# r9y9/gantts

Measured on NVIDIA H100. Metric: gan_step_frames_per_sec, higher is better.
Workload: dtype f32 (GEMMs: bf16x3 split on wgmma, fp32 accumulate)

## Files before the change

### gantts_b200/csrc/common.cuh

```cuda
#pragma once
#include <cuda_runtime.h>
#include <stdint.h>
#include <stdio.h>
#include <stdlib.h>
#include <string.h>

#include "../../include/gantts_b200.h"

namespace gantts {

void set_error(const char* fmt, ...);
int cuda_fail(cudaError_t e, const char* what);

#define GANTTS_CHECK_ARG(cond, ...)            \
  do {                                         \
    if (!(cond)) {                             \
      ::gantts::set_error(__VA_ARGS__);        \
      return GANTTS_E_BADARG;                  \
    }                                          \
  } while (0)

#define GANTTS_CUDA(call)                                        \
  do {                                                           \
    cudaError_t _e = (call);                                     \
    if (_e != cudaSuccess) return ::gantts::cuda_fail(_e, #call); \
  } while (0)

#define GANTTS_LAUNCH_CHECK(name)                                     \
  do {                                                                \
    cudaError_t _e = cudaGetLastError();                              \
    if (_e != cudaSuccess) return ::gantts::cuda_fail(_e, "launch " name); \
    ::gantts::count_launch();                                         \
  } while (0)

void count_launch();
enum ProfKind { PROF_GEMM_KK = 0, PROF_GEMM_MN = 1, PROF_MLPG_FWD = 2, PROF_MLPG_BWD = 3, PROF_LSTM_FWD = 4,
                PROF_LSTM_BWD = 5, PROF_WORLD_RESPONSE = 6, PROF_WORLD_OLA = 7, PROF_KINDS = 8 };
void prof_begin(int kind, double work, cudaStream_t st);
void prof_end(cudaStream_t st);

static inline cudaStream_t as_stream(void* s) { return reinterpret_cast<cudaStream_t>(s); }

int side_stream(cudaStream_t* out);
int stream_wait(cudaStream_t waiter, cudaStream_t on);

__device__ __forceinline__ void pdl_entry() {
  asm volatile("griddepcontrol.launch_dependents;" ::: "memory");
  asm volatile("griddepcontrol.wait;" ::: "memory");
}
inline int pdl_enabled() {
  static int v = -1;
  if (v < 0) {
    const char* e = getenv("GANTTS_B200_PDL");
    v = e ? atoi(e) : 1;
  }
  return v;
}
template <typename... KA, typename... A>
static inline void pdl_launch(void (*kern)(KA...), dim3 grid, dim3 block, size_t smem, cudaStream_t st, A&&... args) {
  cudaLaunchConfig_t cfg = {};
  cfg.gridDim = grid;
  cfg.blockDim = block;
  cfg.dynamicSmemBytes = smem;
  cfg.stream = st;
  cudaLaunchAttribute at[1];
  at[0].id = cudaLaunchAttributeProgrammaticStreamSerialization;
  at[0].val.programmaticStreamSerializationAllowed = 1;
  cfg.attrs = at;
  cfg.numAttrs = pdl_enabled() ? 1 : 0;
  cudaLaunchKernelEx(&cfg, kern, static_cast<KA>(args)...);
}
#define GANTTS_PDL_LAUNCH(kern, grid, block, smem, st, ...) \
  ::gantts::pdl_launch(kern, dim3(grid), dim3(block), (size_t)(smem), st, __VA_ARGS__)

__device__ __forceinline__ float warp_sum(float v) {
#pragma unroll
  for (int o = 16; o > 0; o >>= 1) v += __shfl_xor_sync(0xffffffffu, v, o);
  return v;
}

template <int NV>
__device__ __forceinline__ void block_sum(float (&v)[NV], float* smem) {
  const int lane = threadIdx.x & 31, warp = threadIdx.x >> 5, nwarp = (blockDim.x + 31) >> 5;
#pragma unroll
  for (int i = 0; i < NV; ++i) v[i] = warp_sum(v[i]);
  if (lane == 0) {
#pragma unroll
    for (int i = 0; i < NV; ++i) smem[i * 32 + warp] = v[i];
  }
  __syncthreads();
  if (warp == 0) {
#pragma unroll
    for (int i = 0; i < NV; ++i) {
      float x = lane < nwarp ? smem[i * 32 + lane] : 0.f;
      v[i] = warp_sum(x);
    }
  }
}

__device__ __forceinline__ void fft_radix2_stages(double2* z, const double2* w, int N) {
  for (int h = 1; h < N; h <<= 1) {
    const int step = N / h;
    for (int i = threadIdx.x; i < N / 2; i += blockDim.x) {
      const int pos = i & (h - 1), i0 = ((i - pos) << 1) + pos, i1 = i0 + h;
      const double2 tw = w[pos * step], a = z[i0], v = z[i1];
      const double tr = tw.x * v.x - tw.y * v.y, ti = tw.x * v.y + tw.y * v.x;
      z[i0] = make_double2(a.x + tr, a.y + ti);
      z[i1] = make_double2(a.x - tr, a.y - ti);
    }
    __syncthreads();
  }
}

__device__ __forceinline__ double2 rfft_split(const double2* z, const double2* w, int k, int N) {
  if (k == 0 || k == N)
    return make_double2(k == 0 ? z[0].x + z[0].y : z[0].x - z[0].y, 0.0);
  const double2 a = z[k], c = z[N - k];
  const double er = 0.5 * (a.x + c.x), ei = 0.5 * (a.y - c.y);
  const double orr = 0.5 * (a.y + c.y), oi = -0.5 * (a.x - c.x);
  const double2 tw = w[k];
  return make_double2(er + (tw.x * orr - tw.y * oi), ei + (tw.x * oi + tw.y * orr));
}

struct DropBits {
  uint32_t a, b;
};
__device__ __forceinline__ DropBits dropout_quad_bits(uint64_t seed, uint32_t row, uint32_t quarter_n, uint32_t quad) {
  uint32_t x = (row * quarter_n + quad) * 0x9E3779B1u + static_cast<uint32_t>(seed);
  x ^= x >> 16; x *= 0x7feb352dU; x ^= x >> 15; x *= 0x846ca68bU; x ^= x >> 16;
  uint32_t y = x * 0x9E3779B1u;
  y ^= y >> 15;
  const uint32_t s = static_cast<uint32_t>(seed >> 32);
  DropBits r;
  r.a = x ^ s;
  r.b = y ^ s;
  return r;
}
__device__ __forceinline__ uint32_t drop_limit(uint32_t thresh) { return ((thresh - 1u) << 16) | 0xffffu; }
__device__ __forceinline__ bool dropout_keep(uint64_t seed, uint32_t row, uint32_t n_cols, uint32_t col,
                                             uint32_t thresh) {
  const DropBits q = dropout_quad_bits(seed, row, (n_cols + 3) >> 2, col >> 2);
  const uint32_t w = (col & 2) ? q.b : q.a;
  const uint32_t f = (col & 1) ? (w >> 16) : (w & 0xffffu);
  return f >= thresh;
}

}
```

### gantts_b200/csrc/core.cu

```cuda
#include <stdarg.h>

#include <mutex>
#include <vector>

#include "common.cuh"

namespace gantts {
static thread_local char g_err[512] = "";

void set_error(const char* fmt, ...) {
  va_list ap;
  va_start(ap, fmt);
  vsnprintf(g_err, sizeof(g_err), fmt, ap);
  va_end(ap);
}

int cuda_fail(cudaError_t e, const char* what) {
  set_error("CUDA error %d (%s) in %s", static_cast<int>(e), cudaGetErrorString(e), what);
  return GANTTS_E_CUDA;
}

static long long g_launches = 0;
void count_launch() { ++g_launches; }

struct ProfRec {
  cudaEvent_t e0, e1;
  int kind;
  double work;
};
static bool g_prof_on = false;
static std::vector<ProfRec> g_recs;
static std::vector<cudaEvent_t> g_pool;
static ProfRec g_open;
static bool g_open_valid = false;

static cudaEvent_t get_event() {
  cudaEvent_t e;
  if (!g_pool.empty()) {
    e = g_pool.back();
    g_pool.pop_back();
    return e;
  }
  cudaEventCreate(&e);
  return e;
}

void prof_begin(int kind, double work, cudaStream_t st) {
  if (!g_prof_on) return;
  g_open.e0 = get_event();
  g_open.e1 = get_event();
  g_open.kind = kind;
  g_open.work = work;
  cudaEventRecord(g_open.e0, st);
  g_open_valid = true;
}

void prof_end(cudaStream_t st) {
  if (!g_prof_on || !g_open_valid) return;
  cudaEventRecord(g_open.e1, st);
  g_recs.push_back(g_open);
  g_open_valid = false;
}

struct SideStream {
  cudaStream_t st = nullptr;
  cudaEvent_t ev = nullptr;
};
static std::mutex g_side_mu;
static SideStream g_side[64];

static int side_locked(SideStream** out) {
  int dev = 0;
  GANTTS_CUDA(cudaGetDevice(&dev));
  GANTTS_CHECK_ARG(dev >= 0 && dev < 64, "side stream: device ordinal %d out of range", dev);
  SideStream& s = g_side[dev];
  if (!s.ev) GANTTS_CUDA(cudaEventCreateWithFlags(&s.ev, cudaEventDisableTiming));
  if (!s.st) {
    int least = 0, greatest = 0;
    GANTTS_CUDA(cudaDeviceGetStreamPriorityRange(&least, &greatest));
    GANTTS_CUDA(cudaStreamCreateWithPriority(&s.st, cudaStreamNonBlocking, greatest));
  }
  *out = &s;
  return GANTTS_OK;
}

int side_stream(cudaStream_t* out) {
  std::lock_guard<std::mutex> lk(g_side_mu);
  SideStream* s;
  int rc = side_locked(&s);
  if (rc) return rc;
  *out = s->st;
  return GANTTS_OK;
}

int stream_wait(cudaStream_t waiter, cudaStream_t on) {
  std::lock_guard<std::mutex> lk(g_side_mu);
  SideStream* s;
  int rc = side_locked(&s);
  if (rc) return rc;
  GANTTS_CUDA(cudaEventRecord(s->ev, on));
  GANTTS_CUDA(cudaStreamWaitEvent(waiter, s->ev, 0));
  return GANTTS_OK;
}
}

extern "C" long long gantts_launch_count(void) { return gantts::g_launches; }

extern "C" int gantts_profile_enable(int on) {
  gantts::g_prof_on = on != 0;
  return GANTTS_OK;
}

extern "C" int gantts_profile_collect(double* ms, double* work, long long* launches) {
  using namespace gantts;
  for (auto& r : g_recs) {
    float t = 0.f;
    cudaError_t e = cudaEventSynchronize(r.e1);
    if (e == cudaSuccess) e = cudaEventElapsedTime(&t, r.e0, r.e1);
    if (e != cudaSuccess) return cuda_fail(e, "profile_collect");
    if (r.kind >= 0 && r.kind < PROF_KINDS) {
      if (ms) ms[r.kind] += t;
      if (work) work[r.kind] += r.work;
      if (launches) launches[r.kind] += 1;
    }
    g_pool.push_back(r.e0);
    g_pool.push_back(r.e1);
  }
  g_recs.clear();
  return GANTTS_OK;
}

extern "C" int gantts_version(void) { return 104; }

extern "C" const char* gantts_last_error_string(void) { return gantts::g_err; }

extern "C" int gantts_device_supported(void) {
  int dev = 0;
  if (cudaGetDevice(&dev) != cudaSuccess) return 0;
  cudaDeviceProp prop;
  if (cudaGetDeviceProperties(&prop, dev) != cudaSuccess) return 0;
  return (prop.major == 9 && prop.minor == 0) ? 1 : 0;
}
```

### gantts_b200/csrc/gan_step.cu

```cuda
#include <nvtx3/nvToolsExt.h>

#include "common.cuh"

namespace gantts {

struct NvtxRange {
  explicit NvtxRange(const char* name) { nvtxRangePushA(name); }
  ~NvtxRange() { nvtxRangePop(); }
};

enum ScalarSlot {
  S_REAL = 0,
  S_FAKE = 3,
  S_ADV = 6,
  S_MGE = 9,
  S_MSE = 11,
  S_DSUMSQ = 13,
  S_GSUMSQ = 14,
  S_INV_T = 15,
  S_ADV_SCALE = 16,
  S_MGE_SCALE = 17,
  S_MSE_SCALE = 18,
  S_COUNT = 32
};
// ... 610 lines not shown
    w->c[l] = a.f32((size_t)M * nc);
    if (l < nl - 1) w->h[l] = a.f32((size_t)M * nc);
    w->w[l] = a.take(2 * plane_bytes(ni, ku) + 2 * plane_bytes(ku, ni));
    w->partial[l] = reinterpret_cast<float*>(a.take(mn_partial_bytes_upto(M, ni, ku)));
  }
  w->du = a.take(nl > 0 ? 2 * plane_bytes(M, maxku) : 0);
  w->dx = a.f32((size_t)M * nc);
  w->dxp = a.f32((size_t)M * nc);
  w->bpart = a.f32((size_t)c->B * 2 * nc);
}

static Planes sru_in_planes(const gantts_gan_step_t* c, const StepLayout& L, int l, int64_t M) {
  char* cur = L.sru.in[l];
  return carve_planes(cur, M, sru_nin(c->sru, l));
}
static void sru_w_planes(const gantts_gan_step_t* c, const StepLayout& L, int l, Planes* w, Planes* wt) {
  const int ni = sru_nin(c->sru, l), ku = sru_ncols(c->sru) * sru_k(c->sru, l);
  char* cur = L.sru.w[l];
  *w = carve_planes(cur, ni, ku);
  *wt = carve_planes(cur, ku, ni);
}

static int sru_stack_fwd(const gantts_gan_step_t* c, const gantts_mlp_t& g, const ParamList& pg, const StepLayout& L,
                         const float* x, int B, int T, uint64_t seed, bool train, cudaStream_t st) {
  const int64_t M = (int64_t)B * T;
  const gantts_sru_stack_t& s = c->sru;
  const int nl = s.num_layers, nc = sru_ncols(s);
  const float p_h = train ? s.dropout : 0.f, p_x = train ? s.rnn_dropout : 0.f;
  int rc;
  {
    WeightSplitList wl;
    wl.n = nl;
    wl.off[0] = 0;
    for (int l = 0; l < nl; ++l) {
      Planes w, wt;
      sru_w_planes(c, L, l, &w, &wt);
      wl.W[l] = pg.sru[l][WEIGHT].p;
      wl.N[l] = (int)w.rows;
      wl.K[l] = (int)w.cols;
      wl.hi[l] = w.hi;
      wl.lo[l] = w.lo;
      wl.pitch[l] = w.pitch;
      wl.thi[l] = wt.hi;
      wl.tlo[l] = wt.lo;
      wl.tpitch[l] = wt.pitch;
      wl.off[l + 1] = wl.off[l] + (int64_t)((w.rows + 31) / 32) * ((w.cols + 31) / 32);
    }
    int nb = (int)(wl.off[nl] < num_sms() * 8 ? wl.off[nl] : num_sms() * 8);
    GANTTS_PDL_LAUNCH((split_weights_kernel), nb < 1 ? 1 : nb, 256, 0, st, wl);
    GANTTS_LAUNCH_CHECK("split_weights_kernel(sru)");
  }
  const Planes in0 = sru_in_planes(c, L, 0, M);
  if (p_x > 0.f) {
    GANTTS_PDL_LAUNCH((sru_mask_split_kernel), blocks_1d(M * s.in_dim, 1024), 256, 0, st, x, (int64_t)s.in_dim, M, s.in_dim,
                      T, sru_mask(gantts_sru_mask_seed(seed, 0, 0), p_x), in0.hi, in0.lo, in0.pitch);
    GANTTS_LAUNCH_CHECK("sru_mask_split_kernel");
  } else if ((rc = launch_split(x, s.in_dim, M, s.in_dim, in0, 0, st))) {
    return rc;
  }
  Planes top;
  if ((rc = mlp_tape_input_planes(&g, M, L.g_tape, L.g_tape_bytes, &top))) return rc;
  for (int l = 0; l < nl; ++l) {
    const int k = sru_k(s, l);
    const bool last = l == nl - 1;
    Planes w, wt;
    sru_w_planes(c, L, l, &w, &wt);
    EpiArgs e;
    e.epi = EPI_F32;
    e.C = L.sru.u[l];
    e.ldc = (int64_t)nc * k;
    if ((rc = launch_gemm_kk(sru_in_planes(c, L, l, M), wt, e, st))) return rc;
    const Planes out = last ? top : sru_in_planes(c, L, l + 1, M);
    SruStepFwd p{};
    p.u = L.sru.u[l];
    p.xh = k == 3 ? (l == 0 ? x : L.sru.h[l - 1]) : nullptr;
    p.xh_rs = l == 0 ? s.in_dim : nc;
    p.bias = pg.sru[l][BIAS].p;
    p.c = L.sru.c[l];
    p.h = L.sru.h[l];
    p.hi = out.hi;
    p.lo = out.lo;
    p.pitch = out.pitch;
    p.mh = sru_mask(gantts_sru_mask_seed(seed, l, 1), last ? 0.f : p_h);
    p.mx = sru_mask(gantts_sru_mask_seed(seed, l + 1, 0), last ? 0.f : p_x);
    p.B = B;
    p.T = T;
    p.d = s.hidden;
    p.bidir = s.bidirectional;
    p.act = s.act;
    if ((rc = launch_sru_step_fwd(p, k, st))) return rc;
  }
  return GANTTS_OK;
}

static int sru_stack_bwd(const gantts_gan_step_t* c, const StepLayout& L, const ParamList& pg, const float* x, int B, int T,
                         uint64_t seed, cudaStream_t st) {
  const int64_t M = (int64_t)B * T;
  const gantts_sru_stack_t& s = c->sru;
  const int nl = s.num_layers, nc = sru_ncols(s);
  int rc;
  ReduceList rl;
  for (int l = nl - 1; l >= 0; --l) {
    const int k = sru_k(s, l);
    const bool top = l == nl - 1;
    char* cur = L.sru.du;
    const Planes du = carve_planes(cur, M, (int64_t)nc * k);
    SruStepBwd p{};
    p.u = L.sru.u[l];
    p.xh = k == 3 ? (l == 0 ? x : L.sru.h[l - 1]) : nullptr;
    p.xh_rs = l == 0 ? s.in_dim : nc;
    p.bias = pg.sru[l][BIAS].p;
    p.c = L.sru.c[l];
    p.dx = L.sru.dx;
    p.dxp_in = top ? nullptr : L.sru.dxp;
    p.mxu = sru_mask(gantts_sru_mask_seed(seed, l + 1, 0), top ? 0.f : s.rnn_dropout);
    p.mh = sru_mask(gantts_sru_mask_seed(seed, l, 1), top ? 0.f : s.dropout);
    p.du_hi = du.hi;
    p.du_lo = du.lo;
    p.du_pitch = du.pitch;
    p.dxp_out = (k == 3 && l > 0) ? L.sru.dxp : nullptr;
    p.dbias_part = L.sru.bpart;
    p.B = B;
    p.T = T;
    p.d = s.hidden;
    p.bidir = s.bidirectional;
    p.act = s.act;
    if ((rc = launch_sru_step_bwd(p, k, st))) return rc;
    GANTTS_PDL_LAUNCH((sru_bias_reduce_kernel), (2 * nc + 255) / 256, 256, 0, st, L.sru.bpart, B, 2 * nc, pg.sru[l][BIAS].g);
    GANTTS_LAUNCH_CHECK("sru_bias_reduce_kernel");
    if ((rc = launch_gemm_mn(sru_in_planes(c, L, l, M), du, pg.sru[l][WEIGHT].g, nullptr, 0, L.sru.partial[l], st, &rl))) return rc;
    if (l > 0) {
      Planes w, wt;
      sru_w_planes(c, L, l, &w, &wt);
      EpiArgs e;
      e.epi = EPI_F32;
      e.C = L.sru.dx;
      e.ldc = nc;
      if ((rc = launch_gemm_kk(du, w, e, st))) return rc;
    }
  }
  return flush_reduce(rl, 0, st);
}

static LstmParams lstm_layer_params(const LstmStack& k, int l, const int64_t* lengths, int B, int T) {
  const gantts_lstm_stack_t& s = *k.s;
  LstmParams p{};
  p.W_hh = k.p[l][0][W_HH].p;
  if (s.bidirectional)
    p.W_hh_dir = ((int64_t)reinterpret_cast<uintptr_t>(k.p[l][1][W_HH].p) - (int64_t)reinterpret_cast<uintptr_t>(k.p[l][0][W_HH].p)) /
                 (int64_t)sizeof(float);
  p.lengths = lengths;
  p.h_out = k.w->h[l];
  p.gates = k.w->gates[l];
  p.cells = k.w->cells[l];
  p.bar = k.w->bar;
  p.B = B;
  p.T = T;
  p.H = s.hidden;
  p.ndir = lstm_ndir(s);
  return p;
}

static int lstm_stack_fwd(const LstmStack& k, const float* x, int64_t x_rs, const Planes& top, const int64_t* lengths,
                          int B, int T, uint64_t seed, bool train, cudaStream_t st) {
  const int64_t M = (int64_t)B * T;
  const gantts_lstm_stack_t& s = *k.s;
  const int nl = s.num_layers, H = s.hidden, nd = lstm_ndir(s), G4 = 4 * H, nh = nd * H;
  const float p_drop = train ? s.dropout : 0.f;
  int rc;
  {
    WeightSplitList wl;
    LstmBiasList bl;
    wl.n = bl.n = nl * nd;
    wl.off[0] = 0;
    bl.len = G4;
    for (int l = 0; l < nl; ++l) {
      Planes w, wt;
      lstm_w_planes(k, l, &w, &wt);
      for (int d = 0; d < nd; ++d) {
        const int i = l * nd + d;
        wl.W[i] = k.p[l][d][W_IH].p;
        wl.N[i] = G4;
        wl.K[i] = lstm_nin(s, l);
        wl.hi[i] = w.hi + (int64_t)d * G4 * w.pitch;
        wl.lo[i] = w.lo + (int64_t)d * G4 * w.pitch;
        wl.pitch[i] = w.pitch;
        wl.thi[i] = wt.hi + (int64_t)d * G4;
        wl.tlo[i] = wt.lo + (int64_t)d * G4;
        wl.tpitch[i] = wt.pitch;
        wl.off[i + 1] = wl.off[i] + (int64_t)((G4 + 31) / 32) * ((wl.K[i] + 31) / 32);
        bl.a[i] = k.p[l][d][B_IH].p;
        bl.b[i] = k.p[l][d][B_HH].p;
        bl.out[i] = k.w->bias[l] + (int64_t)d * G4;
      }
    }
    const int nb = (int)(wl.off[wl.n] < num_sms() * 8 ? wl.off[wl.n] : num_sms() * 8);
    GANTTS_PDL_LAUNCH((split_weights_kernel), nb < 1 ? 1 : nb, 256, 0, st, wl);
    GANTTS_LAUNCH_CHECK("split_weights_kernel(lstm)");
    GANTTS_PDL_LAUNCH((lstm_bias_sum_kernel), (bl.n * G4 + 255) / 256, 256, 0, st, bl);
    GANTTS_LAUNCH_CHECK("lstm_bias_sum_kernel");
  }
  if (x && (rc = launch_split(x, x_rs, M, s.in_dim, lstm_in_planes(k, 0, M), 0, st))) return rc;
  for (int l = 0; l < nl; ++l) {
    const bool last = l == nl - 1;
    Planes w, wt;
    lstm_w_planes(k, l, &w, &wt);
    EpiArgs e;
    e.epi = EPI_F32;
    e.C = k.w->xproj;
    e.ldc = (int64_t)nd * G4;
    e.bias = k.w->bias[l];
    if ((rc = launch_gemm_kk(lstm_in_planes(k, l, M), w, e, st))) return rc;
    LstmParams p = lstm_layer_params(k, l, lengths, B, T);
    p.xproj = k.w->xproj;
    if ((rc = lstm_run(false, p, st))) return rc;
    const Planes out = last ? top : lstm_in_planes(k, l + 1, M);
    const float pl = last ? 0.f : p_drop;
    GANTTS_PDL_LAUNCH((lstm_planes_kernel), blocks_1d(M * nh, 1024), 256, 0, st, k.w->h[l], M, nh,
                      k.mask_seed(seed, l), pl > 0.f ? (uint32_t)(pl * 65536.f + 0.5f) : 0u,
                      pl > 0.f ? 1.f / (1.f - pl) : 1.f, out.hi, out.lo, out.pitch);
    GANTTS_LAUNCH_CHECK("lstm_planes_kernel");
  }
  return GANTTS_OK;
}

struct LstmInGrad {
  int64_t row0;
  int col0, cols;
  float* C;
  int64_t ldc;
  int accumulate;
};

static int lstm_stack_bwd(const LstmStack& k, const int64_t* lengths, int B, int T, uint64_t seed, bool param_grads,
                          const LstmInGrad* din, cudaStream_t st) {
  const int64_t M = (int64_t)B * T;
  const gantts_lstm_stack_t& s = *k.s;
  const int nl = s.num_layers, H = s.hidden, nd = lstm_ndir(s), G4 = 4 * H, nh = nd * H;
  int rc;
  char* cur = k.w->dg;
  const Planes dg = carve_planes(cur, M, (int64_t)nd * G4);
  cur = k.w->hp;
  const Planes hp = carve_planes(cur, M, H);
  ReduceList rl;
  for (int l = nl - 1; l >= 0; --l) {
    LstmParams p = lstm_layer_params(k, l, lengths, B, T);
    p.dh_out = k.w->dh;
    p.dxproj = k.w->xproj;
    if ((rc = lstm_run(true, p, st))) return rc;
    if ((rc = launch_split(k.w->xproj, (int64_t)nd * G4, M, nd * G4, dg, 0, st))) return rc;
    const Planes in = lstm_in_planes(k, l, M);
    for (int d = 0; d < nd && param_grads; ++d) {
      Planes dgd = dg;
      dgd.hi += (int64_t)d * G4;
      dgd.lo += (int64_t)d * G4;
      dgd.cols = G4;
      if ((rc = launch_gemm_mn(dgd, in, k.p[l][d][W_IH].g, k.p[l][d][B_IH].g, 0, k.w->part[d][0], st, &rl))) return rc;
      GANTTS_PDL_LAUNCH((lstm_hprev_planes_kernel), blocks_1d(M * H, 1024), 256, 0, st, k.w->h[l], lengths, B, T, H, nd,
                        d, hp.hi, hp.lo, hp.pitch);
      GANTTS_LAUNCH_CHECK("lstm_hprev_planes_kernel");
      if ((rc = launch_gemm_mn(dgd, hp, k.p[l][d][W_HH].g, nullptr, 0, k.w->part[d][1], st, &rl))) return rc;
    }
    if (l > 0) {
      Planes w, wt;
      lstm_w_planes(k, l, &w, &wt);
      EpiArgs e;
      e.epi = EPI_F32;
      e.C = k.w->dh;
      e.ldc = nh;
      if (s.dropout > 0.f) {
        e.act = GANTTS_ACT_LEAKY_DROPOUT;
        e.slope = 1.f;
        e.p = s.dropout;
        e.seed = k.mask_seed(seed, l - 1);
      }
      if ((rc = launch_gemm_kk(dg, wt, e, st))) return rc;
    } else if (din) {
      Planes w, wt;
      lstm_w_planes(k, 0, &w, &wt);
      Planes a = dg;
      a.hi += din->row0 * dg.pitch;
      a.lo += din->row0 * dg.pitch;
      a.rows = M - din->row0;
      wt.hi += (int64_t)din->col0 * wt.pitch;
      wt.lo += (int64_t)din->col0 * wt.pitch;
      wt.rows = din->cols;
      EpiArgs e;
      e.epi = EPI_F32;
      e.C = din->C;
      e.ldc = din->ldc;
      e.accumulate = din->accumulate;
      if ((rc = launch_gemm_kk(a, wt, e, st))) return rc;
    }
    if (!param_grads) continue;
    if ((rc = flush_reduce(rl, 0, st))) return rc;
    for (int d = 0; d < nd; ++d)
      GANTTS_CUDA(cudaMemcpyAsync(k.p[l][d][B_HH].g, k.p[l][d][B_IH].g, (size_t)G4 * sizeof(float), cudaMemcpyDeviceToDevice, st));
  }
  return GANTTS_OK;
}

static bool g_side_bwd(const gantts_gan_step_t* c) { return c->sru.num_layers == 0 && c->lstm.num_layers == 0; }
static bool d_side_bwd(const gantts_gan_step_t* c) { return c->d_lstm.num_layers == 0; }

static void layout(const gantts_gan_step_t* c, char* base, StepLayout* L) {
  const int64_t M = (int64_t)c->B * c->T;
  const int dD = d_in_width(c);
  *L = StepLayout{};
  Arena a{base};
  L->scal = a.f32(S_COUNT);
  L->mask = a.f32((size_t)M);
  L->d_in = a.f32((size_t)2 * M * dD);
  L->d_out = a.f32((size_t)2 * M);
  L->g_dout = a.f32((size_t)2 * M);
  L->g_din = a.f32((size_t)2 * M * dD);
  L->g_static = a.f32((size_t)M * c->n_static);
  L->g_yhat = a.f32((size_t)M * c->g.dims[c->g.num_layers]);
  L->g_grads = a.f32(g_param_count(c));
  L->d_grads = a.f32(d_param_count(c));
  L->g_tape_bytes = gantts_mlp_tape_bytes(&c->g, M);
  L->g_tape = a.take(L->g_tape_bytes);
  L->d_tape_bytes = gantts_mlp_tape_bytes(&c->d, 2 * M);
  L->d_tape = a.take(L->d_tape_bytes);
  const size_t gb = mlp_workspace_bytes(&c->g, M, true, g_side_bwd(c));
  const size_t db = mlp_workspace_bytes(&c->d, 2 * M, true, d_side_bwd(c));
  L->mlp_ws_bytes = gb > db ? gb : db;
  L->mlp_ws = a.take(L->mlp_ws_bytes);
  L->red = reinterpret_cast<RedWs*>(a.take(R_COUNT * sizeof(RedWs)));
  L->opt_partial = a.f32(OPT_MAX_BLOCKS);
  layout_highway(c, M, a, &L->hw);
  layout_sru(c, M, a, &L->sru);
  layout_lstm(c->lstm, M, c->g.dims[c->g.num_layers], 0, a, &L->lstm);
  layout_lstm(c->d_lstm, 2 * M, 0, 2 * (int64_t)c->B, a, &L->d_lstm);
  L->total = (size_t)(a.cur - base) + 256;
}

struct Step {
  const gantts_gan_step_t* c;
  StepLayout L;
  int B, T;
  const float* table;
  gantts_mlp_t g, d;
  ParamList pg, pd;
  const float *x, *y;
  const int64_t* lengths;
  float *y_hat, *y_hat_static;
  int64_t M;
  int d_in, d_out, dD, nS;
  int cond_w, nA;
  bool has_d, has_adv;
  bool train;
  bool adv_window;
  HighwayArgs hwa;
  ColList static_cols, adv_cols, real_cols;
  uint64_t seed;
  void* stream;
  cudaStream_t st;
  cudaStream_t side;
  const HighwayArgs* hw() const { return c->highway.static_dim > 0 ? &hwa : nullptr; }
  bool d_rnn() const { return c->d_lstm.num_layers > 0; }
  LstmStack d_lstm(int which) const { return LstmStack{&c->d_lstm, &L.d_lstm, pd.lstm, which}; }
};

static int step_prologue(const Step& s, float inv_frames, bool zero_norms) {
  const gantts_gan_step_t* c = s.c;
  int rc = gantts_sequence_mask(s.lengths, s.L.mask, s.B, s.T, s.stream);
  if (rc) return rc;
  GANTTS_PDL_LAUNCH((set_scales_kernel), 1, 32, 0, s.st, s.L.scal, inv_frames, s.has_adv ? c->adv_w : 0.f, c->mge_w, c->mse_w,
                    zero_norms ? 1 : 0, s.lengths, s.B, s.T);
  GANTTS_LAUNCH_CHECK("set_scales_kernel");
  return GANTTS_OK;
}

static int step_finalize(const Step& s, float* losses_dev) {
  const gantts_gan_step_t* c = s.c;
  RedCounts cnt{};
  if (s.has_d) cnt.n[R_REAL] = cnt.n[R_FAKE] = bce_blocks(s.M);
  if (s.has_adv) cnt.n[R_ADV] = bce_blocks(s.M);
  cnt.n[R_MGE] = sse_blocks(s.M, s.nS);
  cnt.n[R_MSE] = sse_blocks(s.M, s.d_out);
  GANTTS_PDL_LAUNCH((finalize_losses_kernel), 1, RED_THREADS, 0, s.st, s.L.scal, losses_dev, s.L.red, cnt,
                    s.has_adv ? c->adv_w : 0.f, c->mge_w, c->mse_w, s.has_d ? 1 : 0);
  GANTTS_LAUNCH_CHECK("finalize_losses_kernel");
  return GANTTS_OK;
}

static int generator_fwd(Step& s, bool train) {
  const gantts_gan_step_t* c = s.c;
  const StepLayout& L = s.L;
  const int64_t M = s.M;
  const float* gen_out = s.y_hat;
  int rc;
  if (c->lstm.num_layers > 0) {
    Planes top;
    if ((rc = mlp_tape_input_planes(&s.g, M, L.g_tape, L.g_tape_bytes, &top))) return rc;
    if ((rc = lstm_stack_fwd(g_lstm(c, L, s.pg), s.x, s.d_in, top, s.lengths, s.B, s.T, s.seed, train, s.st))) return rc;
    if ((rc = mlp_fwd_impl(&s.g, nullptr, 0, M, L.lstm.out, s.d_out, L.g_tape, L.g_tape_bytes, s.st, true))) return rc;
    GANTTS_CUDA(cudaMemcpyAsync(s.y_hat, s.x, (size_t)M * s.d_in * sizeof(float), cudaMemcpyDeviceToDevice, s.st));
    gen_out = L.lstm.out;
  } else if (c->sru.num_layers > 0) {
    if ((rc = sru_stack_fwd(c, s.g, s.pg, L, s.x, s.B, s.T, s.seed, train, s.st))) return rc;
    if ((rc = mlp_fwd_impl(&s.g, nullptr, 0, M, s.y_hat, s.d_out, L.g_tape, L.g_tape_bytes, s.st, true))) return rc;
  } else if ((rc = gantts_mlp_fwd(&s.g, s.x, s.d_in, M, s.y_hat, s.d_out, L.g_tape, L.g_tape_bytes, s.st))) {
    return rc;
  }
  if (c->highway.static_dim > 0 && (rc = highway_gate_fwd(c, s.g, s.pg, L, M, s.st))) return rc;
  return mlpg_fwd_impl(gen_out, (int64_t)s.T * s.d_out, s.d_out, s.y_hat_static, (int64_t)s.T * s.nS, s.nS, s.table,
                       &c->streams, &c->windows, s.B, s.T, s.stream, s.hw());
}

static int generator_bwd(Step& s) {
  const gantts_gan_step_t* c = s.c;
  const StepLayout& L = s.L;
  const int64_t M = s.M;
  const int d_out = s.d_out, nS = s.nS;
  const bool sru = c->sru.num_layers > 0, lstm = c->lstm.num_layers > 0;
  const bool mse_grad = c->mse_w != 0.f && !lstm;
  const cudaStream_t side = g_side_bwd(c) ? s.side : nullptr;
  int rc;
  const cudaStream_t mse_st = side && !mse_grad ? side : s.st;
  if (mse_st != s.st && (rc = stream_wait(mse_st, s.st))) return rc;
  if ((rc = launch_sse(s.y_hat, d_out, s.y, d_out, L.mask, M, d_out, L.scal + S_MSE_SCALE, mse_grad ? L.g_yhat : nullptr,
                       d_out, &L.red[R_MSE], mse_st)))
    return rc;
  bool direct = false;
  if (!mse_grad) {
    Planes gp;
    if ((rc = mlp_bwd_gy_planes(&s.g, M, L.mlp_ws, L.mlp_ws_bytes, &gp))) return rc;
    rc = mlpg_bwd_planes(L.g_static, (int64_t)s.T * nS, nS, gp.hi, gp.lo, gp.pitch, s.table, &c->streams,
                         &c->windows, s.B, s.T, s.stream, s.hw());
    if (rc == GANTTS_OK) direct = true;
    else if (rc != GANTTS_E_UNSUPPORTED) return rc;
  }
  if (!direct &&
      (rc = mlpg_bwd_impl(L.g_static, (int64_t)s.T * nS, nS, L.g_yhat, (int64_t)s.T * d_out, d_out, s.table,
                          &c->streams, &c->windows, s.B, s.T, mse_grad ? 1 : 0, s.stream, s.hw())))
    return rc;
  if (c->highway.static_dim > 0 && (rc = highway_gate_bwd(c, s.g, s.pg, L, M, s.st))) return rc;
  float* gx = sru ? L.sru.dx : (lstm ? L.lstm.dh : nullptr);
  const int gx_rs = sru ? sru_ncols(c->sru) : (lstm ? lstm_ndir(c->lstm) * c->lstm.hidden : 0);
  if ((rc = mlp_bwd_impl(&s.g, direct ? nullptr : L.g_yhat, d_out, nullptr, 0, M, L.g_tape, L.g_tape_bytes, gx, gx_rs, 0,
                         s.pg.gW, s.pg.gb, 0, L.mlp_ws, L.mlp_ws_bytes, s.stream, -1, direct, side)))
    return rc;
  if (sru) return sru_stack_bwd(c, L, s.pg, s.x, s.B, s.T, s.seed, s.st);
  if (lstm) return lstm_stack_bwd(g_lstm(c, L, s.pg), s.lengths, s.B, s.T, s.seed, true, nullptr, s.st);
  return GANTTS_OK;
}

static int discriminator_stack_fwd(Step& s, bool stacked, const float* x, const Planes& top) {
  const int64_t* lengths = s.lengths;
  if (stacked) {
    lengths = s.L.d_lstm.lengths;
    for (int half = 0; half < 2; ++half)
      GANTTS_CUDA(cudaMemcpyAsync(s.L.d_lstm.lengths + half * s.B, s.lengths, (size_t)s.B * sizeof(int64_t),
                                  cudaMemcpyDeviceToDevice, s.st));
  }
  return lstm_stack_fwd(s.d_lstm(stacked ? 1 : 2), x, s.dD, top, lengths, stacked ? 2 * s.B : s.B, s.T, s.seed, s.train,
                        s.st);
}

static int discriminator_fwd(Step& s, bool stacked) {
  const StepLayout& L = s.L;
  const int64_t M = s.M, rows = stacked ? 2 * M : M;
  int rc;
  Planes tape_in;
  if ((rc = mlp_tape_input_planes(&s.d, rows, L.d_tape, L.d_tape_bytes, &tape_in))) return rc;
  const Planes din = s.d_rnn() ? lstm_in_planes(s.d_lstm(stacked ? 1 : 2), 0, rows) : tape_in;
  if (!s.cond_w) {
    if (stacked) {
      GANTTS_PDL_LAUNCH((gather_planes_kernel), blocks_1d(2 * M * s.nA, 1024), 256, 0, s.st, s.y, s.d_out, s.real_cols, M,
                        s.y_hat_static, s.nS, s.adv_cols, M, din.hi, din.lo, din.pitch);
      GANTTS_LAUNCH_CHECK("gather_planes_kernel(real|fake)");
    } else {
      ColList none;
      none.n = 0;
      GANTTS_PDL_LAUNCH((gather_planes_kernel), blocks_1d(M * s.nA, 1024), 256, 0, s.st, s.y_hat_static, s.nS, s.adv_cols, M,
                        nullptr, 0, none, 0, din.hi, din.lo, din.pitch);
      GANTTS_LAUNCH_CHECK("gather_planes_kernel(adv)");
    }
    if (s.d_rnn() && (rc = discriminator_stack_fwd(s, stacked, nullptr, tape_in))) return rc;
    return mlp_fwd_impl(&s.d, nullptr, 0, rows, L.d_out, 1, L.d_tape, L.d_tape_bytes, s.stream, true);
  }
  const int dD = s.dD;
  if (stacked) {
    gather_cols_list_kernel<<<blocks_1d(M * s.nA, 1024), 256, 0, s.st>>>(s.y, s.d_out, L.d_in + s.cond_w, dD, s.real_cols, M);
    GANTTS_LAUNCH_CHECK("gather_cols_list_kernel(real)");
    gather_cols_list_kernel<<<blocks_1d(M * s.nA, 1024), 256, 0, s.st>>>(s.y_hat_static, s.nS, L.d_in + M * dD + s.cond_w,
                                                                          dD, s.adv_cols, M);
    GANTTS_LAUNCH_CHECK("gather_cols_list_kernel(fake)");
    for (int64_t half = 0; half < 2; ++half)
      GANTTS_CUDA(cudaMemcpy2DAsync(L.d_in + half * M * dD, (size_t)dD * sizeof(float), s.x, (size_t)s.d_in * sizeof(float),
                                    (size_t)s.cond_w * sizeof(float), (size_t)M, cudaMemcpyDeviceToDevice, s.st));
  }
  if (s.d_rnn()) {
    if ((rc = discriminator_stack_fwd(s, stacked, L.d_in + (stacked ? 0 : M * dD), tape_in))) return rc;
    return mlp_fwd_impl(&s.d, nullptr, 0, rows, L.d_out, 1, L.d_tape, L.d_tape_bytes, s.stream, true);
  }
  return gantts_mlp_fwd(&s.d, L.d_in + (stacked ? 0 : M * dD), dD, rows, L.d_out, 1, L.d_tape, L.d_tape_bytes, s.stream);
}

static int discriminator_bwd(Step& s, bool stacked, bool input_grad = true) {
  const StepLayout& L = s.L;
  const int64_t M = s.M, skip = stacked ? M : 0;
  float* const* gW = stacked ? s.pd.gW : nullptr;
  float* const* gb = stacked ? s.pd.gb : nullptr;
  float* gx = !input_grad ? nullptr : (s.adv_window ? L.g_static + s.adv_cols.c[0] - skip * (int64_t)s.nS : L.g_din);
  int rc;
  if (s.d_rnn()) {
    const LstmStack k = s.d_lstm(stacked ? 1 : 2);
    const int nh = lstm_ndir(s.c->d_lstm) * s.c->d_lstm.hidden;
    if ((rc = mlp_bwd_impl(&s.d, L.g_dout, 1, L.d_out, 1, skip + M, L.d_tape, L.d_tape_bytes, k.w->dh, nh, 0, gW, gb, 0,
                           L.mlp_ws, L.mlp_ws_bytes, s.stream, 0)))
      return rc;
    LstmInGrad din{};
    if (input_grad) {
      const int64_t rs = s.adv_window ? s.nS : s.dD;
      din = LstmInGrad{skip, s.cond_w, s.nA, (s.adv_window ? gx : gx + s.cond_w) + skip * rs, rs, s.adv_window ? 1 : 0};
    }
    if ((rc = lstm_stack_bwd(k, stacked ? L.d_lstm.lengths : s.lengths, stacked ? 2 * s.B : s.B, s.T, s.seed, stacked,
                             input_grad ? &din : nullptr, s.st)))
      return rc;
  } else if ((rc = mlp_bwd_impl(&s.d, L.g_dout, 1, L.d_out, 1, skip + M, L.d_tape, L.d_tape_bytes, gx, s.adv_window ? s.nS : s.dD,
                                skip, gW, gb, 0, L.mlp_ws, L.mlp_ws_bytes, s.stream, s.adv_window ? 1 : -1, false,
                                stacked ? s.side : nullptr))) {
    return rc;
  }
  if (s.adv_window || !input_grad) return GANTTS_OK;
  scatter_cols_list_add_kernel<<<blocks_1d(M * s.nA, 1024), 256, 0, s.st>>>(L.g_din + skip * s.dD + s.cond_w, s.dD,
                                                                             L.g_static, s.nS, s.adv_cols, M);
  GANTTS_LAUNCH_CHECK("scatter_cols_list_add_kernel");
  return GANTTS_OK;
}

}

using namespace gantts;

extern "C" uint64_t gantts_gan_step_seed(uint64_t seed, int which) { return seed * 4 + (uint64_t)which; }

extern "C" uint64_t gantts_sru_mask_seed(uint64_t seed, int layer, int which) {
  return gantts_mlp_layer_seed(gantts_gan_step_seed(seed, 3), 2 * layer + which);
}

extern "C" uint64_t gantts_lstm_mask_seed(uint64_t seed, int layer) {
  return gantts_mlp_layer_seed(gantts_gan_step_seed(seed, 3), 2 * GANTTS_MAX_SRU_LAYERS + layer);
}

extern "C" uint64_t gantts_d_lstm_mask_seed(uint64_t seed, int which, int layer) {
  return gantts_mlp_layer_seed(gantts_gan_step_seed(seed, 3),
                               2 * GANTTS_MAX_SRU_LAYERS + GANTTS_MAX_LSTM_LAYERS * which + layer);
}

extern "C" size_t gantts_gan_step_workspace_bytes(const gantts_gan_step_t* c) {
  if (check_step(c)) return 0;
  StepLayout L;
  layout(c, nullptr, &L);
  return L.total + 256;
}

extern "C" int gantts_gan_step_grad_buffer(const gantts_gan_step_t* c, void* workspace, int which, float** ptr,
                                           int64_t* count) {
  int rc = check_step(c);
  if (rc) return rc;
  GANTTS_CHECK_ARG(workspace && ptr && count, "gan_step_grad_buffer: null pointer");
  StepLayout L;
  layout(c, reinterpret_cast<char*>(al256(reinterpret_cast<uintptr_t>(workspace))), &L);
  *ptr = which == 0 ? L.g_grads : L.d_grads;
  *count = which == 0 ? g_param_count(c) : d_param_count(c);
  return GANTTS_OK;
}

extern "C" int gantts_gan_step(const gantts_gan_step_t* c, int phases, const float* x, const float* y,
                               const int64_t* lengths_dev, float inv_frames, uint64_t seed, float* y_hat,
                               float* y_hat_static, float* losses_dev, void* workspace, size_t workspace_bytes,
                               void* stream) {
  GANTTS_CHECK_ARG(c, "gan_step: null config");
  return gantts_gan_step_shaped(c, c->B, c->T, c->mlpg_table, phases, x, y, lengths_dev, inv_frames, seed, y_hat,
                                y_hat_static, losses_dev, workspace, workspace_bytes, stream);
}

extern "C" int gantts_gan_step_shaped(const gantts_gan_step_t* c, int B, int T, const float* mlpg_table, int phases,
                                      const float* x, const float* y, const int64_t* lengths_dev, float inv_frames,
                                      uint64_t seed, float* y_hat, float* y_hat_static, float* losses_dev, void* workspace,
                                      size_t workspace_bytes, void* stream) {
  int rc = check_step(c);
  if (rc) return rc;
  GANTTS_CHECK_ARG(B >= 1 && B <= c->B, "gan_step_shaped: batch size B = %d must be in [1, configured B = %d]", B, c->B);
  GANTTS_CHECK_ARG(T >= 1 && T <= c->T, "gan_step_shaped: padded length T = %d must be in [1, configured T = %d]", T, c->T);
  GANTTS_CHECK_ARG(mlpg_table, "gan_step_shaped: null MLPG table (it must be gantts_mlpg_table(windows, T) of the call's T)");
  const bool d_only = (phases & GANTTS_STEP_D_ONLY) != 0;
  if (d_only) {
    GANTTS_CHECK_ARG(!(phases & GANTTS_STEP_EVAL),
                     "gan_step: GANTTS_STEP_D_ONLY cannot be combined with GANTTS_STEP_EVAL (the test phase updates nothing)");
    GANTTS_CHECK_ARG(c->w_d > 0.f, "gan_step: GANTTS_STEP_D_ONLY trains the discriminator and needs w_d > 0 (got %g)",
                     (double)c->w_d);
  }
  GANTTS_CHECK_ARG(x && y && lengths_dev && y_hat && y_hat_static && losses_dev, "gan_step: null pointer");
  size_t need = gantts_gan_step_workspace_bytes(c);
  if (!workspace || workspace_bytes < need) {
    set_error("gan_step: workspace too small (%zu < %zu)", workspace_bytes, need);
    return GANTTS_E_WORKSPACE;
  }
  Step s;
  s.c = c;
  s.B = B;
  s.T = T;
  s.table = mlpg_table;
  s.stream = stream;
  s.st = as_stream(stream);
  s.side = nullptr;
  if ((g_side_bwd(c) || d_side_bwd(c)) && (rc = side_stream(&s.side))) return rc;
  layout(c, reinterpret_cast<char*>(al256(reinterpret_cast<uintptr_t>(workspace))), &s.L);
  const StepLayout& L = s.L;
  const int64_t M = s.M = (int64_t)B * T;
  s.x = x;
  s.y = y;
  s.lengths = lengths_dev;
  s.y_hat = y_hat;
  s.y_hat_static = y_hat_static;
  s.seed = seed;
  s.train = !(phases & GANTTS_STEP_EVAL);
  s.d_in = gen_in_width(c);
  s.d_out = c->g.dims[c->g.num_layers];
  s.dD = d_in_width(c);
  const int nS = s.nS = c->n_static;
  s.has_d = c->w_d > 0.f;
  s.has_adv = s.has_d && c->adv_w > 0.f && !d_only;
  s.cond_w = (s.has_d && c->d_conditioned) ? s.d_in : 0;
  s.nA = s.dD - s.cond_w;
  s.g = c->g;
  s.d = c->d;
  g_param_list(c, &s.g, L.g_grads, &s.pg);
  s.pd.n = 0;
  s.pd.total = 0;
  if (s.has_d) d_param_list(c, &s.d, L.d_grads, &s.pd);
  s.hwa = HighwayArgs{};
  if (c->highway.static_dim > 0) {
    char* cur = L.hw.dz;
    const Planes dz = carve_planes(cur, M, nS);
    s.hwa = HighwayArgs{x, s.d_in, L.hw.tx, L.hw.gx, dz.hi, dz.lo, dz.pitch, nS};
  }
  s.static_cols.n = c->n_static_cols;
  for (int i = 0; i < c->n_static_cols; ++i) s.static_cols.c[i] = c->static_cols[i];
  s.adv_cols.n = s.has_d ? c->n_adv : 0;
  for (int i = 0; i < s.adv_cols.n; ++i) s.adv_cols.c[i] = c->adv_cols[i];
  s.adv_window = s.has_d && !s.cond_w && s.adv_cols.n >= 1;
  for (int i = 1; i < s.adv_cols.n; ++i) s.adv_window = s.adv_window && s.adv_cols.c[i] == s.adv_cols.c[0] + i;
  s.real_cols.n = s.adv_cols.n;
  for (int i = 0; i < s.adv_cols.n; ++i) {
    GANTTS_CHECK_ARG(s.adv_cols.c[i] >= 0 && s.adv_cols.c[i] < c->n_static_cols, "gan_step: adversarial column out of range");
    s.real_cols.c[i] = s.static_cols.c[s.adv_cols.c[i]];
  }
  s.g.seed = gantts_gan_step_seed(seed, 0);
  const cudaStream_t st = s.st;

  if (phases & GANTTS_STEP_EVAL) {
    NvtxRange r_eval("gantts_gan_step/eval");
    GANTTS_CHECK_ARG(phases == GANTTS_STEP_EVAL, "gan_step: GANTTS_STEP_EVAL cannot be combined with training phases");
    s.g.dropout_p = 0.f;
    s.d.dropout_p = 0.f;
    if ((rc = step_prologue(s, inv_frames, true))) return rc;
    if ((rc = generator_fwd(s, false))) return rc;
    if (s.has_d) {
      if ((rc = discriminator_fwd(s, true))) return rc;
      if ((rc = launch_bce(L.d_out, L.mask, M, 2, 0, 1, L.scal + S_INV_T, nullptr, &L.red[R_REAL], &L.red[R_FAKE], st)))
        return rc;
      if (s.has_adv &&
          (rc = launch_bce(L.d_out + M, L.mask, M, 1, 0, 0, L.scal + S_INV_T, nullptr, &L.red[R_ADV], nullptr, st)))
        return rc;
    }
    if ((rc = launch_sse(y_hat_static, nS, y, s.d_out, L.mask, M, nS, L.scal + S_MGE_SCALE, nullptr, 0, &L.red[R_MGE], st,
                         &s.static_cols)))
      return rc;
    if ((rc = launch_sse(y_hat, s.d_out, y, s.d_out, L.mask, M, s.d_out, L.scal + S_MSE_SCALE, nullptr, 0, &L.red[R_MSE],
                         st)))
      return rc;
    return step_finalize(s, losses_dev);
  }

  if (phases & 1) {
    NvtxRange r1("gantts_gan_step/phase1: G fwd, MLPG, MGE, D fwd+bwd");
    if ((rc = step_prologue(s, inv_frames, d_only))) return rc;
    if ((rc = generator_fwd(s, true))) return rc;
    if ((rc = launch_sse(y_hat_static, nS, y, s.d_out, L.mask, M, nS, L.scal + S_MGE_SCALE, d_only ? nullptr : L.g_static, nS,
                         &L.red[R_MGE], st, &s.static_cols)))
      return rc;
    if (d_only && (rc = launch_sse(y_hat, s.d_out, y, s.d_out, L.mask, M, s.d_out, L.scal + S_MSE_SCALE, nullptr, 0,
                                   &L.red[R_MSE], st)))
      return rc;
    if (s.has_d) {
      s.d.seed = gantts_gan_step_seed(seed, 1);
      if ((rc = discriminator_fwd(s, true))) return rc;
      if ((rc = launch_bce(L.d_out, L.mask, M, 2, 0, 1, L.scal + S_INV_T, L.g_dout, &L.red[R_REAL], &L.red[R_FAKE], st)))
        return rc;
      if ((rc = discriminator_bwd(s, true, !d_only))) return rc;
    }
  }
  if (d_only) {
    if (phases & 2) {
      NvtxRange r2("gantts_gan_step/phase2 (D only): D step");
      if ((rc = clip_opt_model(c, d_opt_spec(c), s.pd, L.opt_partial, L.scal + S_DSUMSQ, c->lr_d, c->wd_d, st))) return rc;
    }
    if (phases & 4) {
      NvtxRange r4("gantts_gan_step/phase4 (D only): losses");
      return step_finalize(s, losses_dev);
    }
    return GANTTS_OK;
  }
  if (phases & 2) {
    NvtxRange r2("gantts_gan_step/phase2: D step, adv D fwd+bwd, MLPG bwd, G bwd");
    if (s.has_d && (rc = clip_opt_model(c, d_opt_spec(c), s.pd, L.opt_partial, L.scal + S_DSUMSQ, c->lr_d, c->wd_d, st)))
      return rc;
    if (s.has_adv) {
      s.d.seed = gantts_gan_step_seed(seed, 2);
      if ((rc = discriminator_fwd(s, false))) return rc;
      if ((rc = launch_bce(L.d_out, L.mask, M, 1, 0, 0, L.scal + S_ADV_SCALE, L.g_dout, &L.red[R_ADV], nullptr, st)))
        return rc;
      if ((rc = discriminator_bwd(s, false))) return rc;
    }
    if ((rc = generator_bwd(s))) return rc;
  }
  if (phases & 4) {
    NvtxRange r4("gantts_gan_step/phase4: G step, losses");
    if ((rc = clip_opt_model(c, g_opt_spec(c), s.pg, L.opt_partial, L.scal + S_GSUMSQ, c->lr_g, c->wd_g, st))) return rc;
    return step_finalize(s, losses_dev);
  }
  return GANTTS_OK;
}

static int check_spoof_d(const gantts_mlp_t* d, int64_t rows) {
  GANTTS_CHECK_ARG(d, "spoof_count: null reference discriminator");
  GANTTS_CHECK_ARG(d->num_layers >= 1 && d->num_layers <= GANTTS_MAX_LAYERS, "spoof_count: bad layer count %d", d->num_layers);
  GANTTS_CHECK_ARG(d->dims[d->num_layers] == 1 && d->last_act == GANTTS_ACT_SIGMOID,
                   "spoof_count: the reference discriminator must end in a single sigmoid output");
  GANTTS_CHECK_ARG(rows >= 1 && rows < (1 << 24),
                   "spoof_count: B * T = %lld frames, the float count is exact below 2^24", (long long)rows);
  return GANTTS_OK;
}

static int spoof_cols(const char* who, const int* adv_cols, int n_adv, int n_static, int d_width, ColList* cols) {
  GANTTS_CHECK_ARG(n_adv >= 1 && n_adv <= GANTTS_MAX_COLS && n_adv == d_width,
                   "%s: %d adversarial columns != reference discriminator input width %d (it gets no "
                   "linguistic conditioning, train.py:554-555)", who, n_adv, d_width);
  GANTTS_CHECK_ARG(n_static >= 1, "%s: bad n_static", who);
  cols->n = n_adv;
  for (int i = 0; i < n_adv; ++i) {
    GANTTS_CHECK_ARG(adv_cols[i] >= 0 && adv_cols[i] < n_static, "%s: adversarial column %d out of range", who,
                     adv_cols[i]);
    cols->c[i] = adv_cols[i];
  }
  return GANTTS_OK;
}

static int spoof_gather(const float* y_hat_static, int n_static, const ColList& cols, int64_t rows, const Planes& in,
                        cudaStream_t st) {
  ColList none;
  none.n = 0;
  GANTTS_PDL_LAUNCH((gather_planes_kernel), blocks_1d(rows * cols.n, 1024), 256, 0, st, y_hat_static, (int64_t)n_static, cols,
                    rows, nullptr, 0, none, 0, in.hi, in.lo, in.pitch);
  GANTTS_LAUNCH_CHECK("gather_planes_kernel(spoof)");
  return GANTTS_OK;
}

static int spoof_threshold(const float* dout, const int64_t* lengths_dev, int B, int T, float* count_dev, cudaStream_t st) {
  GANTTS_PDL_LAUNCH((spoof_count_kernel), 1, RED_THREADS, 0, st, dout, lengths_dev, B, T, count_dev);
  GANTTS_LAUNCH_CHECK("spoof_count_kernel");
  return GANTTS_OK;
}

extern "C" size_t gantts_spoof_count_workspace_bytes(const gantts_mlp_t* d, int64_t rows) {
  if (check_spoof_d(d, rows)) return 0;
  return al256(gantts_mlp_tape_bytes(d, rows)) + al256((size_t)rows * sizeof(float)) + 256;
}

extern "C" int gantts_spoof_count(const gantts_mlp_t* d, const float* y_hat_static, int n_static, const int* adv_cols,
                                  int n_adv, const int64_t* lengths_dev, int B, int T, float* count_dev, void* ws,
                                  size_t ws_bytes, void* stream) {
  GANTTS_CHECK_ARG(B >= 1 && T >= 1, "spoof_count: bad batch shape");
  const int64_t rows = (int64_t)B * T;
  int rc = check_spoof_d(d, rows);
  if (rc) return rc;
  GANTTS_CHECK_ARG(y_hat_static && adv_cols && lengths_dev && count_dev, "spoof_count: null pointer");
  ColList cols;
  if ((rc = spoof_cols("spoof_count", adv_cols, n_adv, n_static, d->dims[0], &cols))) return rc;
  const size_t need = gantts_spoof_count_workspace_bytes(d, rows);
  if (!ws || ws_bytes < need) {
    set_error("spoof_count: workspace too small (%zu < %zu)", ws_bytes, need);
    return GANTTS_E_WORKSPACE;
  }
  gantts_mlp_t m = *d;
  m.dropout_p = 0.f;
  char* base = reinterpret_cast<char*>(al256(reinterpret_cast<uintptr_t>(ws)));
  const size_t tape_bytes = gantts_mlp_tape_bytes(&m, rows);
  char* tape = base;
  float* dout = reinterpret_cast<float*>(base + al256(tape_bytes));
  const cudaStream_t st = as_stream(stream);
  Planes din;
  if ((rc = mlp_tape_input_planes(&m, rows, tape, tape_bytes, &din))) return rc;
  if ((rc = spoof_gather(y_hat_static, n_static, cols, rows, din, st))) return rc;
  if ((rc = mlp_fwd_impl(&m, nullptr, 0, rows, dout, 1, tape, tape_bytes, stream, true))) return rc;
  return spoof_threshold(dout, lengths_dev, B, T, count_dev, st);
}

struct SpoofLstmLayout {
  LstmWs lstm;
  char* tape;
  size_t tape_bytes;
  float* dout;
  size_t total;
};

static void layout_spoof_lstm(const gantts_lstm_stack_t& ls, const gantts_mlp_t& head, int64_t rows, char* base,
                              SpoofLstmLayout* L) {
  *L = SpoofLstmLayout{};
  Arena a{base};
  layout_lstm(ls, rows, 0, 0, a, &L->lstm, false);
  L->tape_bytes = gantts_mlp_tape_bytes(&head, rows);
  L->tape = a.take(L->tape_bytes);
  L->dout = a.f32((size_t)rows);
  L->total = (size_t)(a.cur - base);
}

static int check_spoof_lstm(const gantts_lstm_stack_t* ls, const gantts_mlp_t* head, int B, int T) {
  GANTTS_CHECK_ARG(ls && head, "spoof_count_lstm: null reference discriminator");
  GANTTS_CHECK_ARG(ls->num_layers >= 1 && ls->num_layers <= GANTTS_MAX_LSTM_LAYERS,
                   "spoof_count_lstm: LSTM layer count %d not in [1, %d] (count with GanTrainer)", ls->num_layers,
                   GANTTS_MAX_LSTM_LAYERS);
  GANTTS_CHECK_ARG(ls->hidden >= 4 && ls->hidden % 4 == 0,
                   "spoof_count_lstm: LSTM hidden size %d is not a positive multiple of 4", ls->hidden);
  GANTTS_CHECK_ARG(ls->bidirectional == 0 || ls->bidirectional == 1, "spoof_count_lstm: bad LSTM bidirectional %d",
                   ls->bidirectional);
  GANTTS_CHECK_ARG(ls->in_dim >= 1, "spoof_count_lstm: bad LSTM in_dim %d", ls->in_dim);
  GANTTS_CHECK_ARG(B >= 1 && T >= 1, "spoof_count_lstm: bad batch shape");
  GANTTS_CHECK_ARG(B <= LSTM_MAX_B, "spoof_count_lstm: an LSTM stack runs at most LSTM_MAX_B = %d sequences (B = %d)",
                   LSTM_MAX_B, B);
  GANTTS_CHECK_ARG((int64_t)B * T < (1 << 24), "spoof_count_lstm: B * T = %lld frames, the float count is exact below 2^24",
                   (long long)B * T);
  const int nh = lstm_ndir(*ls) * ls->hidden;
  GANTTS_CHECK_ARG(head->num_layers == 1 && head->dims[0] == nh && head->dims[1] == 1 && head->last_act == GANTTS_ACT_SIGMOID,
                   "spoof_count_lstm: the head must be hidden2out alone, 1 layer of %d -> 1 with a sigmoid (got %d "
                   "layer(s), input width %d)", nh, head->num_layers, head->dims[0]);
  return GANTTS_OK;
}

extern "C" size_t gantts_spoof_count_lstm_workspace_bytes(const gantts_lstm_stack_t* ls, const gantts_mlp_t* head, int B,
                                                          int T) {
  if (check_spoof_lstm(ls, head, B, T)) return 0;
  SpoofLstmLayout L;
  layout_spoof_lstm(*ls, *head, (int64_t)B * T, nullptr, &L);
  return L.total + 256;
}

extern "C" int gantts_spoof_count_lstm(const gantts_lstm_stack_t* ls, const float* const* lstm_tensors, int n_tensors,
                                       const gantts_mlp_t* head, const float* y_hat_static, int n_static,
                                       const int* adv_cols, int n_adv, const int64_t* lengths_dev, int B, int T,
                                       float* count_dev, void* ws, size_t ws_bytes, void* stream) {
  int rc = check_spoof_lstm(ls, head, B, T);
  if (rc) return rc;
  GANTTS_CHECK_ARG(lstm_tensors && y_hat_static && adv_cols && lengths_dev && count_dev && head->W[0] && head->b[0],
                   "spoof_count_lstm: null pointer");
  const int want = 4 * lstm_ndir(*ls) * ls->num_layers;
  GANTTS_CHECK_ARG(n_tensors == want,
                   "spoof_count_lstm: %d LSTM tensors, the stack has %d (W_ih, W_hh, b_ih, b_hh per layer and direction)",
                   n_tensors, want);
  for (int i = 0; i < n_tensors; ++i) GANTTS_CHECK_ARG(lstm_tensors[i], "spoof_count_lstm: null pointer (LSTM tensor %d)", i);
  ColList cols;
  if ((rc = spoof_cols("spoof_count_lstm", adv_cols, n_adv, n_static, ls->in_dim, &cols))) return rc;
  const size_t need = gantts_spoof_count_lstm_workspace_bytes(ls, head, B, T);
  if (!ws || ws_bytes < need) {
    set_error("spoof_count_lstm: workspace too small (%zu < %zu)", ws_bytes, need);
    return GANTTS_E_WORKSPACE;
  }
  const int64_t rows = (int64_t)B * T;
  SpoofLstmLayout L;
  layout_spoof_lstm(*ls, *head, rows, reinterpret_cast<char*>(al256(reinterpret_cast<uintptr_t>(ws))), &L);
  gantts_step_tensors_t t{};
  t.n = n_tensors;
  for (int i = 0; i < n_tensors; ++i) t.param[i] = const_cast<float*>(lstm_tensors[i]);
  ParamList pl;
  pl.n = 0;
  pl.total = 0;
  bind_lstm(t, *ls, nullptr, &pl);
  const LstmStack k{ls, &L.lstm, pl.lstm, 0};
  gantts_mlp_t m = *head;
  m.dropout_p = 0.f;
  const cudaStream_t st = as_stream(stream);
  if ((rc = spoof_gather(y_hat_static, n_static, cols, rows, lstm_in_planes(k, 0, rows), st))) return rc;
  Planes top;
  if ((rc = mlp_tape_input_planes(&m, rows, L.tape, L.tape_bytes, &top))) return rc;
  if ((rc = lstm_stack_fwd(k, nullptr, 0, top, lengths_dev, B, T, 0, false, st))) return rc;
  if ((rc = mlp_fwd_impl(&m, nullptr, 0, rows, L.dout, 1, L.tape, L.tape_bytes, stream, true))) return rc;
  return spoof_threshold(L.dout, lengths_dev, B, T, count_dev, st);
}
```

### gantts_b200/csrc/gemm_tc.cu

```cuda
#include <cuda.h>
#include <cuda_bf16.h>

#include "common.cuh"
#include "tc_ptx.cuh"

namespace gantts {

constexpr int TC_WG_WARPS = 4;
constexpr int TC_THREADS = 128 + 2 * 32 * TC_WG_WARPS;
constexpr int TC_BM = 128;
constexpr int TC_WARP_PITCH = 20;
constexpr int TC_WARP_BUF_FLOATS = 32 * TC_WARP_PITCH;
constexpr int TC_MAX_BN = 128;
constexpr int TC_KK_BK = 64;
constexpr int TC_MN_BK = 32;
constexpr int TC_MAX_STAGES = 8;
constexpr int TC_PRODUCER_REGS = 40;
constexpr int TC_CONSUMER_REGS = 232;
constexpr uint32_t TC_SMEM_MAX = 227 * 1024;
constexpr uint32_t TC_BIAS_SMEM = 4096;
constexpr uint32_t TC_ONES_SMEM = 1024;

constexpr int EPI_F32 = 0;
constexpr int EPI_PLANES_FWD = 1;
// ... 274 lines not shown
    ptx::wgmma_commit();
    if (kb > 0) {
      ptx::wgmma_wait<1>();
      __syncwarp();
      if (lane == 0) ptx::mbar_arrive(empty0 + 8 * prev);
    }
    prev = s;
    if (++s == (uint32_t)p.num_stages) { s = 0; ph ^= 1; }
  }
  __syncwarp();
  ptx::wgmma_wait<0>();
  ptx::fence_regs(acc);
  ptx::fence_regs(accdb);
  __syncwarp();
  if (lane == 0) ptx::mbar_arrive(empty0 + 8 * prev);
}

template <bool MN, int EPI, int BN>
__global__ void __launch_bounds__(TC_THREADS, 1)
gemm_bf16x3_kernel(const __grid_constant__ CUtensorMap tmAh, const __grid_constant__ CUtensorMap tmAl,
                   const __grid_constant__ CUtensorMap tmBh, const __grid_constant__ CUtensorMap tmBl,
                   const __grid_constant__ CUtensorMap tmOh, const __grid_constant__ CUtensorMap tmOl,
                   const GemmParams p) {
  constexpr int BK = MN ? TC_MN_BK : TC_KK_BK;
  constexpr bool PLANES = EPI != EPI_F32;
  extern __shared__ uint8_t smem_raw[];
  const uint32_t raw = ptx::smem_u32(smem_raw);
  const uint32_t base = (raw + 1023u) & ~1023u;
  uint8_t* const gbase = smem_raw + (base - raw);
  const uint32_t full0 = base + p.bar_off, empty0 = full0 + 8 * TC_MAX_STAGES;
  const int warp = threadIdx.x >> 5, lane = threadIdx.x & 31;
  const int tiles_ab = p.num_a * p.num_b;
  const int tiles = tiles_ab * p.num_z;
  auto k_blocks = [&](int z) {
    const int64_t r_beg = (int64_t)z * p.red_chunk;
    const int64_t r_end = r_beg + p.red_chunk < p.red ? r_beg + p.red_chunk : p.red;
    return (int)((r_end - r_beg + BK - 1) / BK);
  };

  if (threadIdx.x == 0) {
    for (int s = 0; s < p.num_stages; ++s) {
      ptx::mbar_init(full0 + 8 * s, 1);
      ptx::mbar_init(empty0 + 8 * s, 2 * TC_WG_WARPS);
    }
    ptx::fence_barrier_init();
    ptx::prefetch_tensormap(&tmAh);
    ptx::prefetch_tensormap(&tmAl);
    ptx::prefetch_tensormap(&tmBh);
    ptx::prefetch_tensormap(&tmBl);
    if (PLANES) {
      ptx::prefetch_tensormap(&tmOh);
      ptx::prefetch_tensormap(&tmOl);
    }
  }
  ptx::pdl_launch_dependents();
  ptx::pdl_wait();
  const float* bias_s = nullptr;
  if (p.bias_off) {
    float* bs = reinterpret_cast<float*>(gbase + p.bias_off);
    const int nb = p.num_b * BN;
    for (int i = threadIdx.x; i < nb; i += TC_THREADS) bs[i] = i < p.cols_b ? p.bias[i] : 0.f;
    bias_s = bs;
  }
  if (MN && p.db != nullptr) {
    uint32_t* ones = reinterpret_cast<uint32_t*>(gbase + p.ones_off);
    for (int i = threadIdx.x; i < (int)(TC_ONES_SMEM / 4); i += TC_THREADS) ones[i] = 0x3F803F80u;
    ptx::fence_proxy_async();
  }
  __syncthreads();

  if (warp < 4) {
    ptx::setmaxnreg_dec<TC_PRODUCER_REGS>();
    if (threadIdx.x == 0) {
      uint32_t s = 0, ph = 0;
      for (int t = blockIdx.x; t < tiles; t += gridDim.x) {
        const int z = t / tiles_ab, rem = t - z * tiles_ab;
        const int a0 = (rem / p.num_b) * TC_BM, b0 = (rem % p.num_b) * BN;
        const int64_t r_beg = (int64_t)z * p.red_chunk;
        const int nk = k_blocks(z);
        for (int kb = 0; kb < nk; ++kb) {
          const int64_t r0 = r_beg + (int64_t)kb * BK;
          ptx::mbar_wait(empty0 + 8 * s, ph ^ 1);
          const uint32_t fb = full0 + 8 * s;
          ptx::mbar_expect_tx(fb, p.tx_bytes);
          const uint32_t sa_hi = base + s * p.stage_bytes, sa_lo = sa_hi + p.a_plane;
          const uint32_t sb_hi = sa_lo + p.a_plane, sb_lo = sb_hi + p.b_plane_bytes;
          if (!MN) {
            ptx::tma_load_2d(sa_hi, &tmAh, fb, (int32_t)r0, a0);
            ptx::tma_load_2d(sb_hi, &tmBh, fb, (int32_t)r0, b0);
            ptx::tma_load_2d(sa_lo, &tmAl, fb, (int32_t)r0, a0);
            ptx::tma_load_2d(sb_lo, &tmBl, fb, (int32_t)r0, b0);
          } else {
            for (int j = 0; j < TC_BM / 64; ++j) {
              ptx::tma_load_2d(sa_hi + j * p.atom_bytes, &tmAh, fb, a0 + 64 * j, (int32_t)r0);
              ptx::tma_load_2d(sa_lo + j * p.atom_bytes, &tmAl, fb, a0 + 64 * j, (int32_t)r0);
            }
            for (int j = 0; j < BN / 64; ++j) {
              ptx::tma_load_2d(sb_hi + j * p.atom_bytes, &tmBh, fb, b0 + 64 * j, (int32_t)r0);
              ptx::tma_load_2d(sb_lo + j * p.atom_bytes, &tmBl, fb, b0 + 64 * j, (int32_t)r0);
            }
          }
          if (++s == (uint32_t)p.num_stages) { s = 0; ph ^= 1; }
        }
      }
    }
    return;
  }

  ptx::setmaxnreg_inc<TC_CONSUMER_REGS>();
  const int wg = (warp >> 2) - 1;
  const int q = warp & 3;
  float* const wbuf = reinterpret_cast<float*>(gbase + p.epi_off) + (warp - 4) * TC_WARP_BUF_FLOATS;
  const uint64_t d_ones = ptx::make_smem_desc(base + p.ones_off, 0u, 1024u);
  uint32_t s = 0, ph = 0;
  for (int t = blockIdx.x; t < tiles; t += gridDim.x) {
    const int z = t / tiles_ab, rem = t - z * tiles_ab;
    const int nk = k_blocks(z);
    const int ta = rem / p.num_b, tb = rem % p.num_b;
    const int a0 = ta * TC_BM, b0 = tb * BN;
    const int64_t row0 = (int64_t)a0 + 64 * wg + 16 * q;
    const int64_t row = row0 + (lane & 15);
    const bool row_ok = row < p.rows_a;
    constexpr int PASSES = BN / 32;
    uint32_t codes[PASSES];
#pragma unroll
    for (int k = 0; k < PASSES; ++k) {
      const int c = b0 + 16 * (2 * k + (lane >> 4));
      codes[k] = 0u;
      if (EPI == EPI_PLANES_BWD && row_ok && c < p.cols_b) codes[k] = __ldg(p.code + row * p.code_pitch + (c >> 4));
    }
    float acc[BN / 2];
    float accdb[4] = {0.f, 0.f, 0.f, 0.f};
    const bool do_db = MN && p.db != nullptr && tb == 0;
    if (do_db)
      mma_tile<MN, BN, MN>(p, acc, accdb, base, full0, empty0, d_ones, nk, s, ph, lane, wg);
    else
      mma_tile<MN, BN, false>(p, acc, accdb, base, full0, empty0, d_ones, nk, s, ph, lane, wg);
    if (do_db && (lane & 3) == 0) {
      const int64_t r = row0 + (lane >> 2);
      if (r < p.rows_a) p.db[(int64_t)z * p.rows_a + r] = accdb[0];
      if (r + 8 < p.rows_a) p.db[(int64_t)z * p.rows_a + r + 8] = accdb[2];
    }
    uint32_t code_out[PASSES];
    uint32_t hw[8], lw[8];
#pragma unroll
    for (int k = 0; k < PASSES; ++k) {
      code_out[k] = 0u;
      if (PLANES && lane == 0) ptx::bulk_wait_read<0>();
      __syncwarp();
#pragma unroll
      for (int h = 0; h < 2; ++h)
#pragma unroll
        for (int jj = 0; jj < 2; ++jj) {
          const int j = 2 * (2 * k + h) + jj;
          float* w = wbuf + (16 * h + (lane >> 2)) * TC_WARP_PITCH + 8 * jj + 2 * (lane & 3);
          *reinterpret_cast<float2*>(w) = make_float2(acc[4 * j], acc[4 * j + 1]);
          *reinterpret_cast<float2*>(w + 8 * TC_WARP_PITCH) = make_float2(acc[4 * j + 2], acc[4 * j + 3]);
        }
      __syncwarp();
      uint32_t rr[16];
      const float4* src = reinterpret_cast<const float4*>(wbuf + lane * TC_WARP_PITCH);
#pragma unroll
      for (int m = 0; m < 4; ++m) {
        const float4 f = src[m];
        rr[4 * m] = __float_as_uint(f.x); rr[4 * m + 1] = __float_as_uint(f.y);
        rr[4 * m + 2] = __float_as_uint(f.z); rr[4 * m + 3] = __float_as_uint(f.w);
      }
      const int col = b0 + 32 * k;
      const int lcol = col + 16 * (lane >> 4);
      if (EPI == EPI_F32 && !p.vec_ok) {
        __syncwarp();
        if (col < p.cols_b) epilogue_f32_smem(p, rr, row0, lane, col, z, bias_s, wbuf);
      } else if (EPI == EPI_F32) {
        if (row_ok && lcol < p.cols_b) epilogue_chunk16<EPI>(p, rr, row, lcol, z, bias_s, 0u, hw, lw);
      } else {
        if (k > 0) store_planes_pass(&tmOh, &tmOl, wbuf, hw, lw, lane, col - 32, row0, p);
        code_out[k] = epilogue_chunk16<EPI>(p, rr, row, lcol, z, bias_s, codes[k], hw, lw);
      }
    }
    if (PLANES) store_planes_pass(&tmOh, &tmOl, wbuf, hw, lw, lane, b0 + 32 * (PASSES - 1), row0, p);
    if (EPI == EPI_PLANES_FWD && p.code != nullptr && row_ok) {
      uint32_t* cpp = p.code + row * p.code_pitch + (b0 >> 4);
#pragma unroll
      for (int k = 0; k < PASSES; ++k) {
        const int ck = 2 * k + (lane >> 4);
        if (b0 + 16 * ck < p.cols_b) cpp[ck] = code_out[k];
      }
    }
  }
  if (PLANES && lane == 0) ptx::bulk_wait<0>();
}

__global__ void split_planes_kernel(const float* __restrict__ src, int64_t rs, int64_t rows, int cols,
                                    __nv_bfloat16* __restrict__ hi, __nv_bfloat16* __restrict__ lo,
                                    int64_t pitch, int transpose) {
  pdl_entry();
  const int lane = threadIdx.x & 31;
  const int64_t warp = ((int64_t)blockIdx.x * blockDim.x + threadIdx.x) >> 5;
  const int64_t nwarps = ((int64_t)gridDim.x * blockDim.x) >> 5;
  if (!transpose) {
    for (int64_t r = warp; r < rows; r += nwarps) {
      const float* sr = src + r * rs;
      uint32_t* hr = reinterpret_cast<uint32_t*>(hi + r * pitch);
      uint32_t* lr = reinterpret_cast<uint32_t*>(lo + r * pitch);
#pragma unroll 2
      for (int c = 2 * lane; c < cols; c += 64) {
        const float a = sr[c], b = (c + 1 < cols) ? sr[c + 1] : 0.f;
        const uint32_t hp = pack_bf16x2(a, b);
        const float ah = __uint_as_float(hp << 16), bh = __uint_as_float(hp & 0xffff0000u);
        hr[c >> 1] = hp;
        lr[c >> 1] = pack_bf16x2(a - ah, b - bh);
      }
    }
  } else {
    for (int64_t r = warp; r < rows; r += nwarps)
      for (int c = lane; c < cols; c += 32) {
        const float v = src[r * rs + c];
        const __nv_bfloat16 h = __float2bfloat16_rn(v);
        hi[(int64_t)c * pitch + r] = h;
        lo[(int64_t)c * pitch + r] = __float2bfloat16_rn(v - __bfloat162float(h));
      }
  }
}

__global__ void splitk_reduce_kernel(const float* __restrict__ partial, int nsplit, int64_t n,
                                     float* __restrict__ out, int accumulate);

typedef CUresult (*EncodeTiledFn)(CUtensorMap*, CUtensorMapDataType, cuuint32_t, void*, const cuuint64_t*,
                                  const cuuint64_t*, const cuuint32_t*, const cuuint32_t*,
                                  CUtensorMapInterleave, CUtensorMapSwizzle, CUtensorMapL2promotion,
                                  CUtensorMapFloatOOBfill);

static EncodeTiledFn get_encode() {
  static EncodeTiledFn fn = nullptr;
  if (!fn) {
    void* p = nullptr;
    cudaDriverEntryPointQueryResult q;
    if (cudaGetDriverEntryPoint("cuTensorMapEncodeTiled", &p, cudaEnableDefault, &q) == cudaSuccess &&
        q == cudaDriverEntryPointSuccess)
      fn = reinterpret_cast<EncodeTiledFn>(p);
  }
  return fn;
}

static int make_map(CUtensorMap* m, const void* ptr, int64_t rows, int64_t cols, int64_t pitch, int box_rows,
                    int box_cols = 64, CUtensorMapSwizzle swizzle = CU_TENSOR_MAP_SWIZZLE_128B) {
  EncodeTiledFn enc = get_encode();
  if (!enc) {
    set_error("tc: cuTensorMapEncodeTiled entry point unavailable");
    return GANTTS_E_CUDA;
  }
  cuuint64_t dims[2] = {(cuuint64_t)cols, (cuuint64_t)rows};
  cuuint64_t strides[1] = {(cuuint64_t)pitch * 2};
  cuuint32_t box[2] = {(cuuint32_t)box_cols, (cuuint32_t)box_rows};
  cuuint32_t estr[2] = {1, 1};
  CUresult r = enc(m, CU_TENSOR_MAP_DATA_TYPE_BFLOAT16, 2, const_cast<void*>(ptr), dims, strides, box, estr,
                   CU_TENSOR_MAP_INTERLEAVE_NONE, swizzle,
                   CU_TENSOR_MAP_L2_PROMOTION_L2_256B,
                   CU_TENSOR_MAP_FLOAT_OOB_FILL_NONE);
  if (r != CUDA_SUCCESS) {
    set_error("tc: cuTensorMapEncodeTiled failed (%d) rows=%lld cols=%lld pitch=%lld box_rows=%d", (int)r,
              (long long)rows, (long long)cols, (long long)pitch, box_rows);
    return GANTTS_E_CUDA;
  }
  return GANTTS_OK;
}

static int current_device() {
  int dev = -1;
  if (cudaGetDevice(&dev) != cudaSuccess) return -1;
  return dev;
}

static int num_sms() {
  static int n[64] = {};
  const int dev = current_device();
  if (dev < 0 || dev >= 64) return 132;
  if (!n[dev]) {
    cudaDeviceGetAttribute(&n[dev], cudaDevAttrMultiProcessorCount, dev);
    if (n[dev] <= 0) n[dev] = 132;
  }
  return n[dev];
}

static inline int64_t pitch_for(int64_t cols) { return (cols + 15) / 16 * 16; }
static inline size_t plane_bytes(int64_t rows, int64_t cols) {
  return ((size_t)rows * pitch_for(cols) * 2 + 255) / 256 * 256;
}

struct Planes {
  __nv_bfloat16 *hi, *lo;
  int64_t rows, cols, pitch;
};

static Planes carve_planes(char*& cur, int64_t rows, int64_t cols) {
  Planes pl;
  pl.rows = rows;
  pl.cols = cols;
  pl.pitch = pitch_for(cols);
  pl.hi = reinterpret_cast<__nv_bfloat16*>(cur);
  cur += plane_bytes(rows, cols);
  pl.lo = reinterpret_cast<__nv_bfloat16*>(cur);
  cur += plane_bytes(rows, cols);
  return pl;
}

static int launch_split(const float* src, int64_t rs, int64_t rows, int cols, const Planes& pl, int transpose,
                        cudaStream_t st) {
  int64_t total = rows * cols;
  int nb = (int)((total + 1023) / 1024);
  if (nb > num_sms() * 8) nb = num_sms() * 8;
  if (nb < 1) nb = 1;
  GANTTS_PDL_LAUNCH((split_planes_kernel), nb, 256, 0, st, src, rs, rows, cols, pl.hi, pl.lo, pl.pitch, transpose);
  GANTTS_LAUNCH_CHECK("split_planes_kernel");
  return GANTTS_OK;
}

static int pick_bn(int n) {
  int bn = (n + 63) / 64 * 64;
  if (bn <= TC_MAX_BN) return bn;
  int tiles = (n + TC_MAX_BN - 1) / TC_MAX_BN;
  bn = ((n + tiles - 1) / tiles + 63) / 64 * 64;
  return bn;
}

struct EpiArgs {
  int epi = EPI_F32;
  float* C = nullptr;
  int64_t ldc = 0;
  int accumulate = 0;
  __nv_bfloat16 *out_hi = nullptr, *out_lo = nullptr;
  int64_t out_pitch = 0;
  uint32_t* code = nullptr;
  int64_t code_pitch = 0;
  const float* bias = nullptr;
  int act = GANTTS_ACT_NONE;
  float slope = 0.f, p = 0.f;
  uint64_t seed = 0;
  int64_t row0 = 0;
};

static void fill_epilogue(GemmParams& p, const EpiArgs& e) {
  p.C = e.C;
  p.ldc = e.ldc;
  p.accumulate = e.accumulate;
  p.vec_ok = (!e.accumulate && e.C && (e.ldc & 3) == 0 && (reinterpret_cast<uintptr_t>(e.C) & 15) == 0) ? 1 : 0;
  p.out_pitch = e.out_pitch;
  p.code = e.code;
  p.code_pitch = e.code_pitch;
  p.bias = e.bias;
  p.act = e.act;
  p.slope = e.slope;
  p.keep_scale = e.p > 0.f ? 1.f / (1.f - e.p) : 1.f;
  p.thresh = e.p > 0.f ? (uint32_t)(e.p * 65536.f + 0.5f) : 0u;
  p.seed = e.seed;
  p.row0 = e.row0;
}

static size_t plan_smem(GemmParams& p, const EpiArgs& e) {
  const uint32_t epi = 2 * TC_WG_WARPS * TC_WARP_BUF_FLOATS * 4;
  const uint32_t fixed = 1024 + epi + TC_ONES_SMEM + TC_BIAS_SMEM + 256;
  p.num_stages = (int)((TC_SMEM_MAX - fixed) / p.stage_bytes);
  if (p.num_stages > TC_MAX_STAGES) p.num_stages = TC_MAX_STAGES;
  p.epi_off = (uint32_t)p.num_stages * p.stage_bytes;
  p.ones_off = p.epi_off + epi;
  p.bias_off = (e.bias && (size_t)p.num_b * p.bn * sizeof(float) <= TC_BIAS_SMEM) ? p.ones_off + TC_ONES_SMEM : 0u;
  p.bar_off = p.ones_off + TC_ONES_SMEM + TC_BIAS_SMEM;
  return (size_t)p.bar_off + 256 + 1024;
}

template <bool MN, int EPI, int BN>
static int launch_kernel(const CUtensorMap& mAh, const CUtensorMap& mAl, const CUtensorMap& mBh,
                         const CUtensorMap& mBl, const CUtensorMap& mOh, const CUtensorMap& mOl, const GemmParams& p,
                         size_t smem, cudaStream_t st) {
  if (smem > TC_SMEM_MAX) {
    set_error("gemm: shared-memory plan of %zu bytes exceeds %u", smem, TC_SMEM_MAX);
    return GANTTS_E_UNSUPPORTED;
  }
  if (p.num_stages < 2) {
    set_error("gemm: shared-memory plan leaves %d ring stage(s), the mainloop needs 2", p.num_stages);
    return GANTTS_E_UNSUPPORTED;
  }
  static bool attr[64] = {};
  const int dev = current_device();
  if (dev < 0 || dev >= 64 || !attr[dev]) {
    GANTTS_CUDA(cudaFuncSetAttribute(gemm_bf16x3_kernel<MN, EPI, BN>, cudaFuncAttributeMaxDynamicSharedMemorySize,
                                     (int)TC_SMEM_MAX));
    if (dev >= 0 && dev < 64) attr[dev] = true;
  }
  const int tiles = p.num_a * p.num_b * p.num_z;
  const int grid = tiles < num_sms() ? tiles : num_sms();
  prof_begin(MN ? PROF_GEMM_MN : PROF_GEMM_KK, 2.0 * (double)p.rows_a * p.cols_b * (double)p.red, st);
  GANTTS_PDL_LAUNCH((gemm_bf16x3_kernel<MN, EPI, BN>), (unsigned)grid, TC_THREADS, smem, st, mAh, mAl, mBh, mBl, mOh,
                    mOl, p);
  prof_end(st);
  GANTTS_LAUNCH_CHECK("gemm_bf16x3_kernel");
  return GANTTS_OK;
}

template <bool MN, int EPI>
static int launch_bn(const CUtensorMap& mAh, const CUtensorMap& mAl, const CUtensorMap& mBh, const CUtensorMap& mBl,
                     const CUtensorMap& mOh, const CUtensorMap& mOl, const GemmParams& p, size_t smem,
                     cudaStream_t st) {
  if (p.bn == 64) return launch_kernel<MN, EPI, 64>(mAh, mAl, mBh, mBl, mOh, mOl, p, smem, st);
  return launch_kernel<MN, EPI, 128>(mAh, mAl, mBh, mBl, mOh, mOl, p, smem, st);
}

static int launch_gemm_kk(const Planes& A, const Planes& B, const EpiArgs& e, cudaStream_t st) {
  GemmParams p{};
  p.rows_a = A.rows;
  p.cols_b = (int)B.rows;
  p.red = A.cols;
  if (B.cols != A.cols) {
    set_error("gemm_kk: reduction extents differ (%lld vs %lld)", (long long)A.cols, (long long)B.cols);
    return GANTTS_E_BADARG;
  }
  p.a_plane = TC_BM * 128u;
  p.red_chunk = (p.red + TC_KK_BK - 1) / TC_KK_BK * TC_KK_BK;
  p.bn = pick_bn(p.cols_b);
  p.num_a = (int)((p.rows_a + TC_BM - 1) / TC_BM);
  p.num_b = (p.cols_b + p.bn - 1) / p.bn;
  p.num_z = 1;
  p.b_plane_bytes = (uint32_t)p.bn * 128u;
  p.stage_bytes = 2 * p.a_plane + 2 * p.b_plane_bytes;
  p.tx_bytes = p.stage_bytes;
  p.c_zstride = 0;
  fill_epilogue(p, e);
  const size_t smem = plan_smem(p, e);
  CUtensorMap mAh, mAl, mBh, mBl;
  int rc;
  if ((rc = make_map(&mAh, A.hi, A.rows, A.cols, A.pitch, TC_BM))) return rc;
  if ((rc = make_map(&mAl, A.lo, A.rows, A.cols, A.pitch, TC_BM))) return rc;
  if ((rc = make_map(&mBh, B.hi, B.rows, B.cols, B.pitch, p.bn))) return rc;
  if ((rc = make_map(&mBl, B.lo, B.rows, B.cols, B.pitch, p.bn))) return rc;
  if (e.epi == EPI_F32) return launch_bn<false, EPI_F32>(mAh, mAl, mBh, mBl, mAh, mAl, p, smem, st);
  CUtensorMap mOh, mOl;
  if ((rc = make_map(&mOh, e.out_hi, p.rows_a, e.out_pitch, e.out_pitch, 16, 32, CU_TENSOR_MAP_SWIZZLE_NONE))) return rc;
  if ((rc = make_map(&mOl, e.out_lo, p.rows_a, e.out_pitch, e.out_pitch, 16, 32, CU_TENSOR_MAP_SWIZZLE_NONE))) return rc;
  switch (e.epi) {
    case EPI_PLANES_FWD: return launch_bn<false, EPI_PLANES_FWD>(mAh, mAl, mBh, mBl, mOh, mOl, p, smem, st);
    case EPI_PLANES_BWD: return launch_bn<false, EPI_PLANES_BWD>(mAh, mAl, mBh, mBl, mOh, mOl, p, smem, st);
  }
  set_error("gemm_kk: bad epilogue %d", e.epi);
  return GANTTS_E_BADARG;
}

static size_t mn_partial_bytes(int64_t red, int rows_a, int cols_b, int* splits_out, int64_t* chunk_out) {
  int bn = pick_bn(cols_b);
  int tiles = ((rows_a + TC_BM - 1) / TC_BM) * ((cols_b + bn - 1) / bn);
  const int bk = TC_MN_BK;
  int64_t blocks = (red + bk - 1) / bk;
  int64_t splits = num_sms() / tiles;
  if (splits < 1) splits = 1;
  if (splits > blocks) splits = blocks;
  int64_t chunk = (blocks + splits - 1) / splits * bk;
  splits = (red + chunk - 1) / chunk;
  if (splits_out) *splits_out = (int)splits;
  if (chunk_out) *chunk_out = chunk;
  return ((size_t)splits * ((size_t)rows_a * cols_b + rows_a) * sizeof(float) + 255) / 256 * 256;
}

static size_t mn_partial_bytes_upto(int64_t red_max, int rows_a, int cols_b) {
  const int bn = pick_bn(cols_b);
  const int tiles = ((rows_a + TC_BM - 1) / TC_BM) * ((cols_b + bn - 1) / bn);
  const int64_t blocks = (red_max + TC_MN_BK - 1) / TC_MN_BK;
  int64_t splits = num_sms() / tiles;
  if (splits > blocks) splits = blocks;
  if (splits < 1) splits = 1;
  return ((size_t)splits * ((size_t)rows_a * cols_b + rows_a) * sizeof(float) + 255) / 256 * 256;
}

constexpr int REDUCE_MAX_JOBS = 2 * GANTTS_MAX_LAYERS;
struct ReduceList {
  int n = 0;
  const float* partial[REDUCE_MAX_JOBS];
  float* out[REDUCE_MAX_JOBS];
  int splits[REDUCE_MAX_JOBS];
  int64_t len[REDUCE_MAX_JOBS];
  int64_t off[REDUCE_MAX_JOBS + 1];
};

constexpr int MR_WARPS = 8;
__global__ void __launch_bounds__(32 * MR_WARPS) multi_reduce_kernel(ReduceList rl, int accumulate) {
  pdl_entry();
  __shared__ float4 part_s[MR_WARPS][32];
  const int lane = threadIdx.x & 31, w = threadIdx.x >> 5;
  const int64_t total4 = rl.off[rl.n];
  for (int64_t base = (int64_t)blockIdx.x * 32; base < total4; base += (int64_t)gridDim.x * 32) {
    const int64_t i = base + lane;
    int j = 0;
    float4 s = make_float4(0.f, 0.f, 0.f, 0.f);
    int64_t e = 0, n = 0;
    bool vec = false;
    if (i < total4) {
      while (j + 1 < rl.n && i >= rl.off[j + 1]) ++j;
      e = (i - rl.off[j]) * 4;
      n = rl.len[j];
      vec = e + 3 < n && (n & 3) == 0;
      const float* part = rl.partial[j];
      const int splits = rl.splits[j];
      if (vec) {
#pragma unroll 4
        for (int z = w; z < splits; z += MR_WARPS) {
          const float4 v = __ldcg(reinterpret_cast<const float4*>(part + (int64_t)z * n + e));
          s.x += v.x; s.y += v.y; s.z += v.z; s.w += v.w;
        }
      } else {
        for (int z = w; z < splits; z += MR_WARPS) {
          const float* pz = part + (int64_t)z * n + e;
          if (e < n) s.x += pz[0];
          if (e + 1 < n) s.y += pz[1];
          if (e + 2 < n) s.z += pz[2];
          if (e + 3 < n) s.w += pz[3];
        }
      }
    }
    part_s[w][lane] = s;
    __syncthreads();
    if (w == 0 && i < total4) {
      float4 t = part_s[0][lane];
#pragma unroll
      for (int k = 1; k < MR_WARPS; ++k) {
        const float4 v = part_s[k][lane];
        t.x += v.x; t.y += v.y; t.z += v.z; t.w += v.w;
      }
      float* out = rl.out[j];
      if (vec && (reinterpret_cast<uintptr_t>(out) & 15) == 0) {
        float4* o = reinterpret_cast<float4*>(out + e);
        if (accumulate) { const float4 c = *o; t.x += c.x; t.y += c.y; t.z += c.z; t.w += c.w; }
        *o = t;
      } else {
        const float tv[4] = {t.x, t.y, t.z, t.w};
        for (int q = 0; q < 4; ++q)
          if (e + q < n) out[e + q] = accumulate ? out[e + q] + tv[q] : tv[q];
      }
    }
    __syncthreads();
  }
}

static int flush_reduce(ReduceList& rl, int accumulate, cudaStream_t st) {
  if (rl.n == 0) return GANTTS_OK;
  rl.off[0] = 0;
  for (int j = 0; j < rl.n; ++j) rl.off[j + 1] = rl.off[j] + (rl.len[j] + 3) / 4;
  int64_t nb = (rl.off[rl.n] + 31) / 32;
  if (nb > (int64_t)num_sms() * 16) nb = (int64_t)num_sms() * 16;
  GANTTS_PDL_LAUNCH((multi_reduce_kernel), (unsigned)nb, 32 * MR_WARPS, 0, st, rl, accumulate);
  GANTTS_LAUNCH_CHECK("multi_reduce_kernel");
  rl.n = 0;
  return GANTTS_OK;
}

static int launch_gemm_mn(const Planes& A, const Planes& B, float* C, float* gb, int accumulate, float* partial,
                          cudaStream_t st, ReduceList* defer = nullptr) {
  GemmParams p{};
  p.rows_a = A.cols;
  p.cols_b = (int)B.cols;
  p.red = A.rows;
  if (B.rows != A.rows) {
    set_error("gemm_mn: reduction extents differ (%lld vs %lld)", (long long)A.rows, (long long)B.rows);
    return GANTTS_E_BADARG;
  }
  int splits;
  int64_t chunk;
  mn_partial_bytes(p.red, (int)p.rows_a, p.cols_b, &splits, &chunk);
  p.red_chunk = chunk;
  p.num_z = splits;
  p.bn = pick_bn(p.cols_b);
  p.num_a = (int)((p.rows_a + TC_BM - 1) / TC_BM);
  p.num_b = (p.cols_b + p.bn - 1) / p.bn;
  p.atom_bytes = (uint32_t)TC_MN_BK * 128;
  p.a_plane = (TC_BM / 64) * p.atom_bytes;
  p.b_plane_bytes = (uint32_t)(p.bn / 64) * p.atom_bytes;
  p.stage_bytes = 2 * p.a_plane + 2 * p.b_plane_bytes;
  p.tx_bytes = p.stage_bytes;
  const bool direct = (splits == 1 && !accumulate);
  const int64_t n = (int64_t)p.rows_a * p.cols_b;
  float* db_partial = partial + (int64_t)splits * n;
  EpiArgs e;
  e.epi = EPI_F32;
  e.C = direct ? C : partial;
  e.ldc = p.cols_b;
  fill_epilogue(p, e);
  p.c_zstride = n;
  p.db = gb ? (direct ? gb : db_partial) : nullptr;
  const size_t smem = plan_smem(p, e);
  CUtensorMap mAh, mAl, mBh, mBl;
  int rc;
  if ((rc = make_map(&mAh, A.hi, A.rows, A.cols, A.pitch, TC_MN_BK))) return rc;
  if ((rc = make_map(&mAl, A.lo, A.rows, A.cols, A.pitch, TC_MN_BK))) return rc;
  if ((rc = make_map(&mBh, B.hi, B.rows, B.cols, B.pitch, TC_MN_BK))) return rc;
  if ((rc = make_map(&mBl, B.lo, B.rows, B.cols, B.pitch, TC_MN_BK))) return rc;
  if ((rc = launch_bn<true, EPI_F32>(mAh, mAl, mBh, mBl, mAh, mAl, p, smem, st))) return rc;
  if (!direct) {
    if (defer && defer->n + 2 <= REDUCE_MAX_JOBS) {
      int j = defer->n++;
      defer->partial[j] = partial; defer->out[j] = C; defer->splits[j] = splits; defer->len[j] = n;
      if (gb) {
        j = defer->n++;
        defer->partial[j] = db_partial; defer->out[j] = gb; defer->splits[j] = splits; defer->len[j] = p.rows_a;
      }
      return GANTTS_OK;
    }
    splitk_reduce_kernel<<<(unsigned)((n + 1023) / 1024), 256, 0, st>>>(partial, splits, n, C, accumulate);
    GANTTS_LAUNCH_CHECK("splitk_reduce_kernel(tc gW)");
    if (gb) {
// ... 72 lines not shown
```

### gantts_b200/csrc/mlp_tc.cu

```cuda
#include "common.cuh"

namespace gantts {

__global__ void grad_out_to_planes_kernel(const float* __restrict__ gy, int64_t gy_rs,
                                          const float* __restrict__ y, int64_t y_rs, int64_t rows, int cols,
                                          __nv_bfloat16* __restrict__ hi, __nv_bfloat16* __restrict__ lo,
                                          int64_t pitch, int sigmoid) {
  if (cols < 32) {
    const int64_t total = rows * cols;
    for (int64_t i = (int64_t)blockIdx.x * blockDim.x + threadIdx.x; i < total;
         i += (int64_t)gridDim.x * blockDim.x) {
      const int64_t r = i / cols;
      const int c = (int)(i - r * cols);
      float v = gy[r * gy_rs + c];
      if (sigmoid) {
        const float yy = y[r * y_rs + c];
        v *= yy * (1.f - yy);
      }
      const __nv_bfloat16 h = __float2bfloat16_rn(v);
      hi[r * pitch + c] = h;
      lo[r * pitch + c] = __float2bfloat16_rn(v - __bfloat162float(h));
    }
    return;
  }
  const int lane = threadIdx.x & 31;
  const int64_t warp = ((int64_t)blockIdx.x * blockDim.x + threadIdx.x) >> 5;
  const int64_t nwarps = ((int64_t)gridDim.x * blockDim.x) >> 5;
  for (int64_t r = warp; r < rows; r += nwarps)
    for (int c = lane; c < cols; c += 32) {
      float v = gy[r * gy_rs + c];
      if (sigmoid) {
        const float yy = y[r * y_rs + c];
        v *= yy * (1.f - yy);
      }
      const __nv_bfloat16 h = __float2bfloat16_rn(v);
      hi[r * pitch + c] = h;
      lo[r * pitch + c] = __float2bfloat16_rn(v - __bfloat162float(h));
    }
}

__global__ void splitk_reduce_strided_kernel(const float* __restrict__ partial, int nsplit, int stride, int off, int n,
                                             float* __restrict__ out, int accumulate) {
  const int i = blockIdx.x * blockDim.x + threadIdx.x;
  if (i >= n) return;
  float s = 0.f;
  for (int z = 0; z < nsplit; ++z) s += partial[(int64_t)z * stride + off + i];
  out[i] = accumulate ? out[i] + s : s;
}

__global__ void __launch_bounds__(256)
colsum_planes_partial_kernel(const __nv_bfloat16* __restrict__ hi, const __nv_bfloat16* __restrict__ lo,
                             int64_t pitch, int64_t M, int N, int64_t rows_per_chunk,
                             float* __restrict__ partial) {
  __shared__ float sm[8][33];
  const int cx = threadIdx.x & 31, ry = threadIdx.x >> 5;
  const int col = blockIdx.x * 32 + cx;
  const int64_t rbeg = (int64_t)blockIdx.y * rows_per_chunk;
  const int64_t rend = rbeg + rows_per_chunk < M ? rbeg + rows_per_chunk : M;
  float s = 0.f;
  if (col < N)
    for (int64_t r = rbeg + ry; r < rend; r += 8)
      s += __bfloat162float(hi[r * pitch + col]) + __bfloat162float(lo[r * pitch + col]);
  sm[ry][cx] = s;
  __syncthreads();
  if (ry == 0 && col < N) {
    float t = 0.f;
#pragma unroll
    for (int k = 0; k < 8; ++k) t += sm[k][cx];
    partial[(int64_t)blockIdx.y * N + col] = t;
  }
}

struct WeightSplitList {
  int n;
  const float* W[GANTTS_MAX_LAYERS];
  int N[GANTTS_MAX_LAYERS], K[GANTTS_MAX_LAYERS];
  __nv_bfloat16 *hi[GANTTS_MAX_LAYERS], *lo[GANTTS_MAX_LAYERS];
  __nv_bfloat16 *thi[GANTTS_MAX_LAYERS], *tlo[GANTTS_MAX_LAYERS];
  int64_t pitch[GANTTS_MAX_LAYERS], tpitch[GANTTS_MAX_LAYERS];
  int64_t off[GANTTS_MAX_LAYERS + 1];
};

__global__ void __launch_bounds__(256) split_weights_kernel(WeightSplitList wl) {
  pdl_entry();
  __shared__ uint16_t th[32][34], tl[32][34];
  const int cx = threadIdx.x & 31, ry = threadIdx.x >> 5;
  for (int64_t tile = blockIdx.x; tile < wl.off[wl.n]; tile += gridDim.x) {
    int l = 0;
    while (l + 1 < wl.n && tile >= wl.off[l + 1]) ++l;
    const int N = wl.N[l], K = wl.K[l];
    const int tk = (K + 31) / 32;
    const int64_t tt = tile - wl.off[l];
    const int r0 = (int)(tt / tk) * 32, c0 = (int)(tt % tk) * 32;
#pragma unroll
    for (int i = 0; i < 4; ++i) {
      const int r = r0 + ry + 8 * i, c = c0 + cx;
      uint16_t hb = 0, lb = 0;
      if (r < N && c < K) {
        const float v = wl.W[l][(int64_t)r * K + c];
        const __nv_bfloat16 h = __float2bfloat16_rn(v);
        const __nv_bfloat16 lo = __float2bfloat16_rn(v - __bfloat162float(h));
        wl.hi[l][r * wl.pitch[l] + c] = h;
        wl.lo[l][r * wl.pitch[l] + c] = lo;
        hb = __bfloat16_as_ushort(h);
        lb = __bfloat16_as_ushort(lo);
      }
      th[ry + 8 * i][cx] = hb;
      tl[ry + 8 * i][cx] = lb;
    }
    __syncthreads();
#pragma unroll
    for (int i = 0; i < 4; ++i) {
      const int c = c0 + ry + 8 * i, r = r0 + cx;
      if (c < K && r < N) {
        wl.thi[l][(int64_t)c * wl.tpitch[l] + r] = __ushort_as_bfloat16(th[cx][ry + 8 * i]);
        wl.tlo[l][(int64_t)c * wl.tpitch[l] + r] = __ushort_as_bfloat16(tl[cx][ry + 8 * i]);
      }
    }
    __syncthreads();
  }
}

constexpr int GEMV_THREADS = 256;
constexpr int GEMV_MAX_K = 1024;

__global__ void __launch_bounds__(GEMV_THREADS)
gemv_fwd_kernel(const __nv_bfloat16* __restrict__ hi, const __nv_bfloat16* __restrict__ lo, int64_t pitch,
                const float* __restrict__ w, const float* __restrict__ b, float* __restrict__ y, int64_t y_rs,
                int64_t M, int K, int sigmoid) {
  __shared__ float ws[GEMV_MAX_K];
  for (int i = threadIdx.x; i < K; i += GEMV_THREADS) ws[i] = w[i];
  __syncthreads();
  const int lane = threadIdx.x & 31;
  const int64_t warp = ((int64_t)blockIdx.x * GEMV_THREADS + threadIdx.x) >> 5;
  const int64_t nwarps = ((int64_t)gridDim.x * GEMV_THREADS) >> 5;
  const float bias = b[0];
  for (int64_t r = warp; r < M; r += nwarps) {
    const uint32_t* hr = reinterpret_cast<const uint32_t*>(hi + r * pitch);
    const uint32_t* lr = reinterpret_cast<const uint32_t*>(lo + r * pitch);
    float acc = 0.f;
    for (int c = 2 * lane; c < K; c += 64) {
      const uint32_t h2 = hr[c >> 1], l2 = lr[c >> 1];
      const float a0 = __uint_as_float(h2 << 16) + __uint_as_float(l2 << 16);
      const float a1 = __uint_as_float(h2 & 0xffff0000u) + __uint_as_float(l2 & 0xffff0000u);
      acc = fmaf(a0, ws[c], acc);
      if (c + 1 < K) acc = fmaf(a1, ws[c + 1], acc);
    }
    acc = warp_sum(acc);
    if (lane == 0) {
      float z = acc + bias;
      y[r * y_rs] = sigmoid ? 1.f / (1.f + expf(-z)) : z;
    }
  }
}

__global__ void __launch_bounds__(GEMV_THREADS)
gemv_bwd_kernel(const float* __restrict__ gy, int64_t gy_rs, const float* __restrict__ y, int64_t y_rs,
                const __nv_bfloat16* __restrict__ hi, const __nv_bfloat16* __restrict__ lo, int64_t pitch,
                const uint32_t* __restrict__ code, int64_t code_pitch, const float* __restrict__ w,
                __nv_bfloat16* __restrict__ ghi, __nv_bfloat16* __restrict__ glo, int64_t gpitch,
                float* __restrict__ partial, int64_t M, int K, int sigmoid, float dpos, float dneg, float dzero,
                int want_gw) {
  __shared__ float ws[GEMV_MAX_K];
  __shared__ float gws[GEMV_THREADS / 32][GEMV_MAX_K + 1];
  for (int i = threadIdx.x; i < K; i += GEMV_THREADS) ws[i] = w[i];
  const int lane = threadIdx.x & 31, wid = threadIdx.x >> 5;
  for (int i = lane; i <= K; i += 32) gws[wid][i] = 0.f;
  __syncthreads();
  const int64_t warp = ((int64_t)blockIdx.x * GEMV_THREADS + threadIdx.x) >> 5;
  const int64_t nwarps = ((int64_t)gridDim.x * GEMV_THREADS) >> 5;
  float gsum = 0.f;
  for (int64_t r = warp; r < M; r += nwarps) {
    float g = gy[r * gy_rs];
    if (sigmoid) {
      const float yy = y[r * y_rs];
      g *= yy * (1.f - yy);
    }
    gsum += g;
    const uint32_t* hr = reinterpret_cast<const uint32_t*>(hi + r * pitch);
    const uint32_t* lr = reinterpret_cast<const uint32_t*>(lo + r * pitch);
    uint32_t* gh = reinterpret_cast<uint32_t*>(ghi + r * gpitch);
    uint32_t* gl = reinterpret_cast<uint32_t*>(glo + r * gpitch);
    for (int c = 2 * lane; c < K; c += 64) {
      if (want_gw) {
        const uint32_t h2 = hr[c >> 1], l2 = lr[c >> 1];
        const float a0 = __uint_as_float(h2 << 16) + __uint_as_float(l2 << 16);
        const float a1 = __uint_as_float(h2 & 0xffff0000u) + __uint_as_float(l2 & 0xffff0000u);
        gws[wid][c] = fmaf(g, a0, gws[wid][c]);
        if (c + 1 < K) gws[wid][c + 1] = fmaf(g, a1, gws[wid][c + 1]);
      }
      const uint32_t cw = code[r * code_pitch + (c >> 4)];
      const uint32_t c0 = (cw >> (2 * (c & 15))) & 3u, c1 = (cw >> (2 * ((c + 1) & 15))) & 3u;
      const float v0 = g * ws[c] * ((c0 & 1u) ? dzero : ((c0 & 2u) ? dneg : dpos));
      const float v1 = (c + 1 < K) ? g * ws[c + 1] * ((c1 & 1u) ? dzero : ((c1 & 2u) ? dneg : dpos)) : 0.f;
      const uint32_t hp = pack_bf16x2(v0, v1);
      gh[c >> 1] = hp;
      gl[c >> 1] = pack_bf16x2(v0 - __uint_as_float(hp << 16), v1 - __uint_as_float(hp & 0xffff0000u));
    }
  }
  if (want_gw) {
    if (lane == 0) gws[wid][K] = gsum;
    __syncthreads();
    for (int i = threadIdx.x; i <= K; i += GEMV_THREADS) {
      float s = 0.f;
#pragma unroll
      for (int q = 0; q < GEMV_THREADS / 32; ++q) s += gws[q][i];
      partial[(int64_t)blockIdx.x * (K + 1) + i] = s;
    }
  }
}

__device__ __forceinline__ void unpack8(const uint4& h, const uint4& l, float (&a)[8]) {
  const uint32_t hh[4] = {h.x, h.y, h.z, h.w}, ll[4] = {l.x, l.y, l.z, l.w};
#pragma unroll
  for (int i = 0; i < 4; ++i) {
    a[2 * i] = __uint_as_float(hh[i] << 16) + __uint_as_float(ll[i] << 16);
    a[2 * i + 1] = __uint_as_float(hh[i] & 0xffff0000u) + __uint_as_float(ll[i] & 0xffff0000u);
  }
}

__device__ __forceinline__ uint4 ldg_stream16(const void* p) {
  uint4 v;
  asm volatile("ld.global.nc.L1::no_allocate.v4.u32 {%0,%1,%2,%3}, [%4];"
               : "=r"(v.x), "=r"(v.y), "=r"(v.z), "=r"(v.w)
               : "l"(p));
  return v;
}

template <int NCH, int RU>
__global__ void __launch_bounds__(GEMV_THREADS)
gemv_fwd_vec_kernel(const __nv_bfloat16* __restrict__ hi, const __nv_bfloat16* __restrict__ lo, int64_t pitch,
                    const float* __restrict__ w, const float* __restrict__ b, float* __restrict__ y, int64_t y_rs,
                    int64_t M, int K, int sigmoid) {
  pdl_entry();
  const int lane = threadIdx.x & 31;
  float wr[NCH][8];
#pragma unroll
  for (int ch = 0; ch < NCH; ++ch) {
    const int c = ch * 256 + lane * 8;
#pragma unroll
    for (int j = 0; j < 8; ++j) wr[ch][j] = c < K ? w[c + j] : 0.f;
  }
  const int64_t warp = ((int64_t)blockIdx.x * GEMV_THREADS + threadIdx.x) >> 5;
  const int64_t nwarps = ((int64_t)gridDim.x * GEMV_THREADS) >> 5;
  const float bias = b[0];
  for (int64_t r0 = warp * RU; r0 < M; r0 += nwarps * RU) {
    uint4 h[RU][NCH], l[RU][NCH];
#pragma unroll
    for (int u = 0; u < RU; ++u) {
      const int64_t r = r0 + u < M ? r0 + u : M - 1;
#pragma unroll
      for (int ch = 0; ch < NCH; ++ch) {
        const int c = ch * 256 + lane * 8;
        if (c < K) {
          h[u][ch] = ldg_stream16(hi + r * pitch + c);
          l[u][ch] = ldg_stream16(lo + r * pitch + c);
        } else {
          h[u][ch] = make_uint4(0, 0, 0, 0);
          l[u][ch] = make_uint4(0, 0, 0, 0);
        }
      }
    }
    float acc[RU];
#pragma unroll
    for (int u = 0; u < RU; ++u) {
      acc[u] = 0.f;
#pragma unroll
      for (int ch = 0; ch < NCH; ++ch) {
        float a[8];
        unpack8(h[u][ch], l[u][ch], a);
#pragma unroll
        for (int j = 0; j < 8; ++j) acc[u] = fmaf(a[j], wr[ch][j], acc[u]);
      }
    }
#pragma unroll
    for (int u = 0; u < RU; ++u) acc[u] = warp_sum(acc[u]);
    if (lane == 0) {
#pragma unroll
      for (int u = 0; u < RU; ++u)
        if (r0 + u < M) {
          const float z = acc[u] + bias;
          y[(r0 + u) * y_rs] = sigmoid ? 1.f / (1.f + expf(-z)) : z;
        }
    }
  }
}

template <int NCH, int RU>
__global__ void __launch_bounds__(GEMV_THREADS)
gemv_bwd_vec_kernel(const float* __restrict__ gy, int64_t gy_rs, const float* __restrict__ y, int64_t y_rs,
                    const __nv_bfloat16* __restrict__ hi, const __nv_bfloat16* __restrict__ lo, int64_t pitch,
                    const uint32_t* __restrict__ code, int64_t code_pitch, const float* __restrict__ w,
                    __nv_bfloat16* __restrict__ ghi, __nv_bfloat16* __restrict__ glo, int64_t gpitch,
                    float* __restrict__ partial, int64_t M, int K, int sigmoid, float dpos, float dneg, float dzero,
                    int want_gw) {
  pdl_entry();
  __shared__ float gws[GEMV_THREADS / 32][GEMV_MAX_K + 1];
  const int lane = threadIdx.x & 31, wid = threadIdx.x >> 5;
  float wr[NCH][8], gw[NCH][8];
#pragma unroll
  for (int ch = 0; ch < NCH; ++ch) {
    const int c = ch * 256 + lane * 8;
#pragma unroll
    for (int j = 0; j < 8; ++j) {
      wr[ch][j] = c < K ? w[c + j] : 0.f;
      gw[ch][j] = 0.f;
    }
  }
  const int64_t warp = ((int64_t)blockIdx.x * GEMV_THREADS + threadIdx.x) >> 5;
  const int64_t nwarps = ((int64_t)gridDim.x * GEMV_THREADS) >> 5;
  float gsum = 0.f;
  for (int64_t r0 = warp * RU; r0 < M; r0 += nwarps * RU) {
    uint4 h[RU][NCH], l[RU][NCH];
    uint32_t cw[RU][NCH];
    float g[RU];
#pragma unroll
    for (int u = 0; u < RU; ++u) {
      const bool ok = r0 + u < M;
      const int64_t r = ok ? r0 + u : M - 1;
      float gg = ok ? gy[r * gy_rs] : 0.f;
      if (sigmoid) {
        const float yy = y[r * y_rs];
        gg *= yy * (1.f - yy);
      }
      g[u] = gg;
#pragma unroll
      for (int ch = 0; ch < NCH; ++ch) {
        const int c = ch * 256 + lane * 8;
        if (c < K) {
          if (want_gw) {
            h[u][ch] = ldg_stream16(hi + r * pitch + c);
            l[u][ch] = ldg_stream16(lo + r * pitch + c);
          }
          cw[u][ch] = __ldg(code + r * code_pitch + (c >> 4)) >> (2 * (c & 15));
        }
      }
    }
#pragma unroll
    for (int u = 0; u < RU; ++u) {
      gsum += g[u];
      if (r0 + u >= M) continue;
      const int64_t r = r0 + u;
#pragma unroll
      for (int ch = 0; ch < NCH; ++ch) {
        const int c = ch * 256 + lane * 8;
        if (c >= K) continue;
        if (want_gw) {
          float a[8];
          unpack8(h[u][ch], l[u][ch], a);
#pragma unroll
          for (int j = 0; j < 8; ++j) gw[ch][j] = fmaf(g[u], a[j], gw[ch][j]);
        }
        uint32_t oh[4], ol[4];
#pragma unroll
        for (int j = 0; j < 4; ++j) {
          const uint32_t c0 = (cw[u][ch] >> (4 * j)) & 3u, c1 = (cw[u][ch] >> (4 * j + 2)) & 3u;
          const float v0 = g[u] * wr[ch][2 * j] * ((c0 & 1u) ? dzero : ((c0 & 2u) ? dneg : dpos));
          const float v1 = g[u] * wr[ch][2 * j + 1] * ((c1 & 1u) ? dzero : ((c1 & 2u) ? dneg : dpos));
          oh[j] = pack_bf16x2(v0, v1);
          ol[j] = pack_bf16x2(v0 - __uint_as_float(oh[j] << 16), v1 - __uint_as_float(oh[j] & 0xffff0000u));
        }
        *reinterpret_cast<uint4*>(ghi + r * gpitch + c) = make_uint4(oh[0], oh[1], oh[2], oh[3]);
        *reinterpret_cast<uint4*>(glo + r * gpitch + c) = make_uint4(ol[0], ol[1], ol[2], ol[3]);
      }
    }
  }
  if (want_gw) {
#pragma unroll
    for (int ch = 0; ch < NCH; ++ch) {
      const int c = ch * 256 + lane * 8;
      if (c < K) {
#pragma unroll
        for (int j = 0; j < 8; ++j) gws[wid][c + j] = gw[ch][j];
      }
    }
    if (lane == 0) gws[wid][K] = gsum;
    __syncthreads();
    for (int i = threadIdx.x; i <= K; i += GEMV_THREADS) {
      float s = 0.f;
#pragma unroll
      for (int q = 0; q < GEMV_THREADS / 32; ++q) s += gws[q][i];
      partial[(int64_t)blockIdx.x * (K + 1) + i] = s;
    }
  }
}

__global__ void __launch_bounds__(256)
gemv_partial_reduce_kernel(const float* __restrict__ partial, int blocks, int K, float* __restrict__ out_w,
                           float* __restrict__ out_b, int accumulate) {
  pdl_entry();
  __shared__ float sm[8][33];
  const int cl = threadIdx.x & 31, rg = threadIdx.x >> 5;
  const int c = blockIdx.x * 32 + cl;
  float s = 0.f;
  if (c <= K)
    for (int b = rg; b < blocks; b += 8) s += partial[(int64_t)b * (K + 1) + c];
  sm[rg][cl] = s;
  __syncthreads();
  if (rg == 0 && c <= K) {
    float t = 0.f;
#pragma unroll
    for (int q = 0; q < 8; ++q) t += sm[q][cl];
    float* o = c < K ? (out_w ? out_w + c : nullptr) : out_b;
    if (o) *o = accumulate ? *o + t : t;
  }
}

constexpr int GEMV_BLOCKS = 132 * 2;

constexpr int MLP_COLSUM_CHUNKS = 128;
constexpr int MLP_GRAD_BUFS = 2;

static int colsum_planes(const Planes& G, float* gb, int accumulate, float* partial, cudaStream_t st) {
  int chunks = MLP_COLSUM_CHUNKS;
  int64_t rpc = (G.rows + chunks - 1) / chunks;
  if (rpc < 8) rpc = 8;
  chunks = (int)((G.rows + rpc - 1) / rpc);
  dim3 grid((unsigned)((G.cols + 31) / 32), chunks);
  colsum_planes_partial_kernel<<<grid, 256, 0, st>>>(G.hi, G.lo, G.pitch, G.rows, (int)G.cols, rpc, partial);
  GANTTS_LAUNCH_CHECK("colsum_planes_partial_kernel");
  splitk_reduce_kernel<<<(unsigned)((G.cols + 1023) / 1024), 256, 0, st>>>(partial, chunks, G.cols, gb, accumulate);
  GANTTS_LAUNCH_CHECK("splitk_reduce_kernel(colsum planes)");
  return GANTTS_OK;
}

struct MlpTape {
  uint32_t* code[GANTTS_MAX_LAYERS];
  int64_t code_pitch[GANTTS_MAX_LAYERS];
  Planes H[GANTTS_MAX_LAYERS];
  Planes W[GANTTS_MAX_LAYERS];
  Planes Wt[GANTTS_MAX_LAYERS];
};

static int check_mlp(const gantts_mlp_t* m, int64_t M) {
  GANTTS_CHECK_ARG(m, "mlp: null descriptor");
  GANTTS_CHECK_ARG(m->num_layers >= 1 && m->num_layers <= GANTTS_MAX_LAYERS, "mlp: bad layer count %d", m->num_layers);
  GANTTS_CHECK_ARG(M >= 1, "mlp: M must be >= 1");
  for (int l = 0; l <= m->num_layers; ++l) GANTTS_CHECK_ARG(m->dims[l] >= 1, "mlp: bad dim[%d]", l);
  for (int l = 0; l < m->num_layers; ++l) {
    GANTTS_CHECK_ARG(m->W[l] && m->b[l], "mlp: null weight/bias of layer %d", l);
    GANTTS_CHECK_ARG((reinterpret_cast<uintptr_t>(m->b[l]) & 15) == 0, "mlp: bias %d must be 16-byte aligned", l);
  }
  GANTTS_CHECK_ARG(m->dropout_p >= 0.f && m->dropout_p < 1.f, "mlp: dropout p out of [0,1)");
  GANTTS_CHECK_ARG(m->last_act == GANTTS_ACT_NONE || m->last_act == GANTTS_ACT_SIGMOID, "mlp: bad last_act");
  return GANTTS_OK;
}

static size_t carve_tape(const gantts_mlp_t* m, int64_t M, char* base, MlpTape* t) {
  char* cur = base;
  for (int l = 0; l < m->num_layers; ++l) {
    Planes p = carve_planes(cur, M, m->dims[l]);
    if (t) t->H[l] = p;
    const int64_t cp = ((m->dims[l] + 15) / 16 + 3) / 4 * 4;
    if (t) {
      t->code[l] = reinterpret_cast<uint32_t*>(cur);
      t->code_pitch[l] = cp;
    }
    if (l >= 1) cur += ((size_t)M * cp * sizeof(uint32_t) + 255) / 256 * 256;
  }
  for (int l = 0; l < m->num_layers; ++l) {
    Planes a = carve_planes(cur, m->dims[l + 1], m->dims[l]);
    Planes b = carve_planes(cur, m->dims[l], m->dims[l + 1]);
    if (t) { t->W[l] = a; t->Wt[l] = b; }
  }
  return (size_t)(cur - base);
}

static inline uint64_t layer_seed(uint64_t seed, int l) { return seed + 0x9E3779B97F4A7C15ull * (uint64_t)(l + 1); }

}

using namespace gantts;

extern "C" uint64_t gantts_mlp_layer_seed(uint64_t seed, int layer) { return layer_seed(seed, layer); }

extern "C" size_t gantts_mlp_tape_bytes(const gantts_mlp_t* m, int64_t M) {
  if (!m || m->num_layers < 1 || m->num_layers > GANTTS_MAX_LAYERS || M < 1) return 0;
  return carve_tape(m, M, nullptr, nullptr) + 512;
}

namespace gantts {
static int mlp_grad_bufs(const gantts_mlp_t* m, bool side) {
  return side && m->num_layers > MLP_GRAD_BUFS ? m->num_layers : MLP_GRAD_BUFS;
}

static size_t mlp_workspace_bytes(const gantts_mlp_t* m, int64_t M, bool upto, bool side = false) {
  if (!m || m->num_layers < 1 || m->num_layers > GANTTS_MAX_LAYERS || M < 1) return 0;
  int maxd = 0;
  size_t part = 0;
  for (int l = 0; l <= m->num_layers; ++l) maxd = m->dims[l] > maxd ? m->dims[l] : maxd;
  for (int l = 0; l < m->num_layers; ++l)
    part += (upto ? mn_partial_bytes_upto(M, m->dims[l + 1], m->dims[l])
                  : mn_partial_bytes(M, m->dims[l + 1], m->dims[l], nullptr, nullptr)) + 256;
  return (size_t)2 * mlp_grad_bufs(m, side) * plane_bytes(M, maxd) + part +
         (size_t)MLP_COLSUM_CHUNKS * maxd * sizeof(float) + (size_t)GEMV_BLOCKS * (GEMV_MAX_K + 1) * sizeof(float) + 4096;
}
}

extern "C" size_t gantts_mlp_workspace_bytes(const gantts_mlp_t* m, int64_t M) { return mlp_workspace_bytes(m, M, false); }

namespace gantts {
static int mlp_fwd_impl(const gantts_mlp_t* m, const float* x, int64_t x_rs, int64_t M, float* y, int64_t y_rs, void* tape,
                        size_t tape_bytes, void* stream, bool input_ready);

static int mlp_tape_input_planes(const gantts_mlp_t* m, int64_t M, void* tape, size_t tape_bytes, Planes* out) {
  int rc = check_mlp(m, M);
  if (rc) return rc;
  if (!tape || tape_bytes < gantts_mlp_tape_bytes(m, M)) {
    set_error("mlp_tape_input_planes: tape too small");
    return GANTTS_E_WORKSPACE;
  }
  MlpTape t;
  carve_tape(m, M, reinterpret_cast<char*>((reinterpret_cast<uintptr_t>(tape) + 255) / 256 * 256), &t);
  *out = t.H[0];
  return GANTTS_OK;
}
}

extern "C" int gantts_mlp_fwd(const gantts_mlp_t* m, const float* x, int64_t x_rs, int64_t M, float* y,
                              int64_t y_rs, void* tape, size_t tape_bytes, void* stream) {
  GANTTS_CHECK_ARG(m && x && x_rs >= m->dims[0], "mlp_fwd: bad input pointer/stride");
  return mlp_fwd_impl(m, x, x_rs, M, y, y_rs, tape, tape_bytes, stream, false);
}

static int gantts::mlp_fwd_impl(const gantts_mlp_t* m, const float* x, int64_t x_rs, int64_t M, float* y, int64_t y_rs,
                                void* tape, size_t tape_bytes, void* stream, bool input_ready) {
  int rc = check_mlp(m, M);
  if (rc) return rc;
  GANTTS_CHECK_ARG((x || input_ready) && y && y_rs >= m->dims[m->num_layers], "mlp_fwd: bad pointers/strides");
  size_t need = gantts_mlp_tape_bytes(m, M);
  if (!tape || tape_bytes < need) {
    set_error("mlp_fwd: tape too small (%zu < %zu)", tape_bytes, need);
    return GANTTS_E_WORKSPACE;
  }
  cudaStream_t st = as_stream(stream);
  MlpTape t;
  carve_tape(m, M, reinterpret_cast<char*>((reinterpret_cast<uintptr_t>(tape) + 255) / 256 * 256), &t);
  const int L = m->num_layers;
  if (!input_ready && (rc = launch_split(x, x_rs, M, m->dims[0], t.H[0], 0, st))) return rc;
  {
    WeightSplitList wl;
    wl.n = L;
    wl.off[0] = 0;
    for (int l = 0; l < L; ++l) {
      wl.W[l] = m->W[l];
      wl.N[l] = m->dims[l + 1];
      wl.K[l] = m->dims[l];
      wl.hi[l] = t.W[l].hi;
      wl.lo[l] = t.W[l].lo;
      wl.pitch[l] = t.W[l].pitch;
      wl.thi[l] = t.Wt[l].hi;
      wl.tlo[l] = t.Wt[l].lo;
      wl.tpitch[l] = t.Wt[l].pitch;
      wl.off[l + 1] = wl.off[l] + (int64_t)((m->dims[l + 1] + 31) / 32) * ((m->dims[l] + 31) / 32);
    }
    int nb = (int)wl.off[L];
    if (nb > num_sms() * 8) nb = num_sms() * 8;
    if (nb < 1) nb = 1;
    GANTTS_PDL_LAUNCH((split_weights_kernel), nb, 256, 0, st, wl);
    GANTTS_LAUNCH_CHECK("split_weights_kernel");
  }
  for (int l = 0; l < L; ++l) {
    EpiArgs e;
    e.bias = m->b[l];
    if (l < L - 1) {
      e.epi = EPI_PLANES_FWD;
      e.out_hi = t.H[l + 1].hi;
      e.out_lo = t.H[l + 1].lo;
      e.out_pitch = t.H[l + 1].pitch;
      e.code = t.code[l + 1];
      e.code_pitch = t.code_pitch[l + 1];
      e.act = GANTTS_ACT_LEAKY_DROPOUT;
      e.slope = m->slope;
      e.p = m->dropout_p;
      e.seed = layer_seed(m->seed, l);
    } else {
      if (m->dims[L] == 1 && L >= 2 && m->dims[l] <= GEMV_MAX_K && (m->dims[l] & 1) == 0) {
        const int Kl = m->dims[l], sg = m->last_act == GANTTS_ACT_SIGMOID;
        if (Kl % 8 == 0 && Kl <= 256)
          GANTTS_PDL_LAUNCH((gemv_fwd_vec_kernel<1, 4>), 2 * GEMV_BLOCKS, GEMV_THREADS, 0, st, t.H[l].hi, t.H[l].lo, t.H[l].pitch, m->W[l],
                                                                          m->b[l], y, y_rs, M, Kl, sg);
        else if (Kl % 8 == 0 && Kl <= 512)
          gemv_fwd_vec_kernel<2, 2><<<2 * GEMV_BLOCKS, GEMV_THREADS, 0, st>>>(t.H[l].hi, t.H[l].lo, t.H[l].pitch, m->W[l],
                                                                          m->b[l], y, y_rs, M, Kl, sg);
        else if (Kl % 8 == 0)
          gemv_fwd_vec_kernel<4, 1><<<2 * GEMV_BLOCKS, GEMV_THREADS, 0, st>>>(t.H[l].hi, t.H[l].lo, t.H[l].pitch, m->W[l],
                                                                          m->b[l], y, y_rs, M, Kl, sg);
        else
          gemv_fwd_kernel<<<GEMV_BLOCKS, GEMV_THREADS, 0, st>>>(t.H[l].hi, t.H[l].lo, t.H[l].pitch, m->W[l], m->b[l], y,
                                                                y_rs, M, Kl, sg);
        GANTTS_LAUNCH_CHECK("gemv_fwd_kernel");
        continue;
      }
      e.epi = EPI_F32;
      e.C = y;
      e.ldc = y_rs;
      e.act = m->last_act;
    }
    if ((rc = launch_gemm_kk(t.H[l], t.W[l], e, st))) return rc;
  }
  return GANTTS_OK;
}

namespace gantts {
static int mlp_bwd_impl(const gantts_mlp_t* m, const float* gy, int64_t gy_rs, const float* y, int64_t y_rs, int64_t M,
                        const void* tape, size_t tape_bytes, float* gx, int64_t gx_rs, int64_t gx_row0,
                        float* const* gW, float* const* gb, int accumulate, void* workspace, size_t workspace_bytes,
                        void* stream, int gx_accumulate = -1, bool gy_planes_ready = false, cudaStream_t side = nullptr);
static int mlp_bwd_gy_planes(const gantts_mlp_t* m, int64_t M, void* workspace, size_t workspace_bytes, Planes* out);
}

static int gantts::mlp_bwd_gy_planes(const gantts_mlp_t* m, int64_t M, void* workspace, size_t workspace_bytes, Planes* out) {
  int rc = check_mlp(m, M);
  if (rc) return rc;
  if (!workspace || workspace_bytes < gantts_mlp_workspace_bytes(m, M)) {
    set_error("mlp_bwd_gy_planes: workspace too small");
    return GANTTS_E_WORKSPACE;
  }
  char* cur = reinterpret_cast<char*>((reinterpret_cast<uintptr_t>(workspace) + 255) / 256 * 256);
  *out = carve_planes(cur, M, m->dims[m->num_layers]);
  return GANTTS_OK;
}

extern "C" int gantts_mlp_bwd(const gantts_mlp_t* m, const float* gy, int64_t gy_rs, const float* y,
                              int64_t y_rs, int64_t M, const void* tape, size_t tape_bytes, float* gx,
                              int64_t gx_rs, float* const* gW, float* const* gb, int accumulate,
                              void* workspace, size_t workspace_bytes, void* stream) {
  return mlp_bwd_impl(m, gy, gy_rs, y, y_rs, M, tape, tape_bytes, gx, gx_rs, 0, gW, gb, accumulate, workspace,
                      workspace_bytes, stream, -1);
}

static int gantts::mlp_bwd_impl(const gantts_mlp_t* m, const float* gy, int64_t gy_rs, const float* y, int64_t y_rs,
                                int64_t M, const void* tape, size_t tape_bytes, float* gx, int64_t gx_rs,
                                int64_t gx_row0, float* const* gW, float* const* gb, int accumulate, void* workspace,
                                size_t workspace_bytes, void* stream, int gx_accumulate, bool gy_planes_ready,
                                cudaStream_t side) {
  if (gx_accumulate < 0) gx_accumulate = accumulate;
  int rc = check_mlp(m, M);
  GANTTS_CHECK_ARG(gx_row0 >= 0 && gx_row0 < M, "mlp_bwd: bad gx_row0");
  if (rc) return rc;
  const int L = m->num_layers;
  GANTTS_CHECK_ARG(gy_planes_ready || (gy && gy_rs >= m->dims[L]), "mlp_bwd: bad gy");
  GANTTS_CHECK_ARG(!gy_planes_ready || (m->last_act == GANTTS_ACT_NONE && m->dims[L] > 1),
                   "mlp_bwd: gy planes are only accepted for a linear multi-column output");
  GANTTS_CHECK_ARG(m->last_act != GANTTS_ACT_SIGMOID || y, "mlp_bwd: sigmoid output needs y");
  if (!tape || tape_bytes < gantts_mlp_tape_bytes(m, M)) {
    set_error("mlp_bwd: tape too small");
    return GANTTS_E_WORKSPACE;
  }
  size_t need = mlp_workspace_bytes(m, M, false, side != nullptr);
  if (!workspace || workspace_bytes < need) {
    set_error("mlp_bwd: workspace too small (%zu < %zu)", workspace_bytes, need);
    return GANTTS_E_WORKSPACE;
  }
  cudaStream_t st = as_stream(stream);
  const cudaStream_t ws = side ? side : st;
  auto fork = [&]() { return side ? stream_wait(side, st) : GANTTS_OK; };
  MlpTape t;
  carve_tape(m, M, reinterpret_cast<char*>((reinterpret_cast<uintptr_t>(const_cast<void*>(tape)) + 255) / 256 * 256), &t);
  int maxd = 0;
  for (int l = 0; l <= L; ++l) maxd = m->dims[l] > maxd ? m->dims[l] : maxd;
  char* cur = reinterpret_cast<char*>((reinterpret_cast<uintptr_t>(workspace) + 255) / 256 * 256);
  const int nbuf = mlp_grad_bufs(m, side != nullptr);
  char* gbuf[GANTTS_MAX_LAYERS > MLP_GRAD_BUFS ? GANTTS_MAX_LAYERS : MLP_GRAD_BUFS];
  for (int i = 0; i < nbuf; ++i) {
    gbuf[i] = cur;
    cur += 2 * plane_bytes(M, maxd);
  }
  float* colpart = reinterpret_cast<float*>(cur);
  cur += ((size_t)MLP_COLSUM_CHUNKS * maxd * sizeof(float) + 255) / 256 * 256;
  char* partial_cur = cur;
  ReduceList rl;

  float* gemv_part = reinterpret_cast<float*>(partial_cur);
  partial_cur += ((size_t)GEMV_BLOCKS * (GEMV_MAX_K + 1) * sizeof(float) + 255) / 256 * 256;
  int pp = 0;
  int l_start = L - 1;
  char* c0 = gbuf[pp];
  Planes G = carve_planes(c0, M, m->dims[L]);
  if (m->dims[L] == 1 && L >= 2 && m->dims[L - 1] <= GEMV_MAX_K && (m->dims[L - 1] & 1) == 0) {
    const int K1 = m->dims[L - 1];
    char* cg = gbuf[pp];
    G = carve_planes(cg, M, K1);
    const float ks = m->dropout_p > 0.f ? 1.f / (1.f - m->dropout_p) : 1.f;
    const int want = (gW && gW[L - 1]) || (gb && gb[L - 1]);
#define GANTTS_GEMV_BWD_ARGS                                                                                     \
  gy, gy_rs, y, y_rs, t.H[L - 1].hi, t.H[L - 1].lo, t.H[L - 1].pitch, t.code[L - 1], t.code_pitch[L - 1],       \
      m->W[L - 1], G.hi, G.lo, G.pitch, gemv_part, M, K1, m->last_act == GANTTS_ACT_SIGMOID ? 1 : 0, ks,        \
      m->slope * ks, m->dropout_p > 0.f ? 0.f : m->slope, want
    if (K1 % 8 == 0 && K1 <= 256)
      GANTTS_PDL_LAUNCH((gemv_bwd_vec_kernel<1, 4>), GEMV_BLOCKS, GEMV_THREADS, 0, st, GANTTS_GEMV_BWD_ARGS);
    else if (K1 % 8 == 0 && K1 <= 512)
      gemv_bwd_vec_kernel<2, 2><<<GEMV_BLOCKS, GEMV_THREADS, 0, st>>>(GANTTS_GEMV_BWD_ARGS);
    else if (K1 % 8 == 0)
      gemv_bwd_vec_kernel<4, 1><<<GEMV_BLOCKS, GEMV_THREADS, 0, st>>>(GANTTS_GEMV_BWD_ARGS);
    else
      gemv_bwd_kernel<<<GEMV_BLOCKS, GEMV_THREADS, 0, st>>>(GANTTS_GEMV_BWD_ARGS);
#undef GANTTS_GEMV_BWD_ARGS
    GANTTS_LAUNCH_CHECK("gemv_bwd_kernel");
    if (want) {
      if ((rc = fork())) return rc;
      GANTTS_PDL_LAUNCH((gemv_partial_reduce_kernel), (K1 + 1 + 31) / 32, 256, 0, ws, gemv_part, GEMV_BLOCKS, K1,
                                                                    gW ? gW[L - 1] : nullptr,
                                                                    gb ? gb[L - 1] : nullptr, accumulate);
      GANTTS_LAUNCH_CHECK("gemv_partial_reduce_kernel");
    }
    l_start = L - 2;
  } else if (!gy_planes_ready) {
    int64_t total = M * m->dims[L];
    int nb = (int)((total + 1023) / 1024);
    if (nb > num_sms() * 8) nb = num_sms() * 8;
    if (nb < 1) nb = 1;
    grad_out_to_planes_kernel<<<nb, 256, 0, st>>>(gy, gy_rs, y, y_rs, M, m->dims[L], G.hi, G.lo, G.pitch,
                                                  m->last_act == GANTTS_ACT_SIGMOID ? 1 : 0);
    GANTTS_LAUNCH_CHECK("grad_out_to_planes_kernel");
  }
  for (int l = l_start; l >= 0; --l) {
    float* gbl = (gb && gb[l]) ? gb[l] : nullptr;
    if (((gW && gW[l]) || gbl) && (rc = fork())) return rc;
    if (gW && gW[l]) {
      float* partial = reinterpret_cast<float*>(partial_cur);
      partial_cur += mn_partial_bytes(M, m->dims[l + 1], m->dims[l], nullptr, nullptr) + 256;
      if ((rc = launch_gemm_mn(G, t.H[l], gW[l], gbl, accumulate, partial, ws, &rl))) return rc;
    } else if (gbl) {
      if ((rc = colsum_planes(G, gbl, accumulate, colpart, ws))) return rc;
    }
    if (l > 0) {
      char* c1 = gbuf[(pp + 1) % nbuf];
      Planes Gn = carve_planes(c1, M, m->dims[l]);
      EpiArgs e;
      e.epi = EPI_PLANES_BWD;
      e.out_hi = Gn.hi;
      e.out_lo = Gn.lo;
      e.out_pitch = Gn.pitch;
      e.code = t.code[l];
      e.code_pitch = t.code_pitch[l];
      e.slope = m->slope;
      e.p = m->dropout_p;
      if ((rc = launch_gemm_kk(G, t.Wt[l], e, st))) return rc;
      G = Gn;
      pp = (pp + 1) % nbuf;
    } else if (gx) {
      EpiArgs e;
      e.epi = EPI_F32;
      e.C = gx + gx_row0 * gx_rs;
      e.ldc = gx_rs;
      e.accumulate = gx_accumulate;
      Planes Gs = G;
      Gs.hi += gx_row0 * G.pitch;
      Gs.lo += gx_row0 * G.pitch;
      Gs.rows = G.rows - gx_row0;
      if ((rc = launch_gemm_kk(Gs, t.Wt[0], e, st))) return rc;
    }
  }
  if ((rc = flush_reduce(rl, accumulate, ws))) return rc;
  return side ? stream_wait(st, side) : GANTTS_OK;
}
```

Before: 16.46 million.

## Run discriminator real-half forward/backward on a branch stream concurrent with generator

Splits the stacked discriminator pass into real and fake halves. The real half (weight split, forward, BCE, and the backward chain through the MLP down to the first layer) now starts on a new low-priority branch stream before the generator forward, so it overlaps generator work. The fake half runs after the generator, with its backward chain limited to the fake rows. The weight-gradient GEMMs still cover both halves on the side stream once the branch is joined. This adds a third stream, more launches and extra row-window plumbing, and the real-half work may compete with the generator kernels for SMs.

```diff
diff --git a/gantts_b200/csrc/common.cuh b/gantts_b200/csrc/common.cuh
--- a/gantts_b200/csrc/common.cuh
+++ b/gantts_b200/csrc/common.cuh
@@ -42,6 +42,7 @@
 static inline cudaStream_t as_stream(void* s) { return reinterpret_cast<cudaStream_t>(s); }
 
 int side_stream(cudaStream_t* out);
+int branch_stream(cudaStream_t* out);
 int stream_wait(cudaStream_t waiter, cudaStream_t on);
 
 __device__ __forceinline__ void pdl_entry() {
diff --git a/gantts_b200/csrc/core.cu b/gantts_b200/csrc/core.cu
--- a/gantts_b200/csrc/core.cu
+++ b/gantts_b200/csrc/core.cu
@@ -64,6 +64,7 @@
 
 struct SideStream {
   cudaStream_t st = nullptr;
+  cudaStream_t branch = nullptr;
   cudaEvent_t ev = nullptr;
 };
 static std::mutex g_side_mu;
@@ -80,6 +81,11 @@
     GANTTS_CUDA(cudaDeviceGetStreamPriorityRange(&least, &greatest));
     GANTTS_CUDA(cudaStreamCreateWithPriority(&s.st, cudaStreamNonBlocking, greatest));
   }
+  if (!s.branch) {
+    int least = 0, greatest = 0;
+    GANTTS_CUDA(cudaDeviceGetStreamPriorityRange(&least, &greatest));
+    GANTTS_CUDA(cudaStreamCreateWithPriority(&s.branch, cudaStreamNonBlocking, least));
+  }
   *out = &s;
   return GANTTS_OK;
 }
@@ -90,6 +96,15 @@
   int rc = side_locked(&s);
   if (rc) return rc;
   *out = s->st;
+  return GANTTS_OK;
+}
+
+int branch_stream(cudaStream_t* out) {
+  std::lock_guard<std::mutex> lk(g_side_mu);
+  SideStream* s;
+  int rc = side_locked(&s);
+  if (rc) return rc;
+  *out = s->branch;
   return GANTTS_OK;
 }
 
diff --git a/gantts_b200/csrc/gan_step.cu b/gantts_b200/csrc/gan_step.cu
--- a/gantts_b200/csrc/gan_step.cu
+++ b/gantts_b200/csrc/gan_step.cu
@@ -936,6 +936,7 @@
 
 static bool g_side_bwd(const gantts_gan_step_t* c) { return c->sru.num_layers == 0 && c->lstm.num_layers == 0; }
 static bool d_side_bwd(const gantts_gan_step_t* c) { return c->d_lstm.num_layers == 0; }
+static bool d_real_branch(const gantts_gan_step_t* c) { return g_side_bwd(c) && d_side_bwd(c); }
 
 static void layout(const gantts_gan_step_t* c, char* base, StepLayout* L) {
   const int64_t M = (int64_t)c->B * c->T;
@@ -991,6 +992,7 @@
   void* stream;
   cudaStream_t st;
   cudaStream_t side;
+  cudaStream_t branch;
   const HighwayArgs* hw() const { return c->highway.static_dim > 0 ? &hwa : nullptr; }
   bool d_rnn() const { return c->d_lstm.num_layers > 0; }
   LstmStack d_lstm(int which) const { return LstmStack{&c->d_lstm, &L.d_lstm, pd.lstm, which}; }
@@ -1093,38 +1095,50 @@
                         s.st);
 }
 
-static int discriminator_fwd(Step& s, bool stacked) {
+static int discriminator_fwd(Step& s, bool stacked, int half = -1) {
   const StepLayout& L = s.L;
   const int64_t M = s.M, rows = stacked ? 2 * M : M;
+  const int64_t r0 = half == 1 ? M : 0, r1 = half == 0 ? M : rows;
   int rc;
   Planes tape_in;
   if ((rc = mlp_tape_input_planes(&s.d, rows, L.d_tape, L.d_tape_bytes, &tape_in))) return rc;
   const Planes din = s.d_rnn() ? lstm_in_planes(s.d_lstm(stacked ? 1 : 2), 0, rows) : tape_in;
+  ColList none;
+  none.n = 0;
   if (!s.cond_w) {
-    if (stacked) {
+    if (stacked && half < 0) {
       GANTTS_PDL_LAUNCH((gather_planes_kernel), blocks_1d(2 * M * s.nA, 1024), 256, 0, s.st, s.y, s.d_out, s.real_cols, M,
                         s.y_hat_static, s.nS, s.adv_cols, M, din.hi, din.lo, din.pitch);
       GANTTS_LAUNCH_CHECK("gather_planes_kernel(real|fake)");
+    } else if (half == 0) {
+      GANTTS_PDL_LAUNCH((gather_planes_kernel), blocks_1d(M * s.nA, 1024), 256, 0, s.st, s.y, s.d_out, s.real_cols, M,
+                        nullptr, 0, none, 0, din.hi, din.lo, din.pitch);
+      GANTTS_LAUNCH_CHECK("gather_planes_kernel(real)");
     } else {
-      ColList none;
-      none.n = 0;
+      const Planes fk = plane_rows(din, r0, r0 + M);
       GANTTS_PDL_LAUNCH((gather_planes_kernel), blocks_1d(M * s.nA, 1024), 256, 0, s.st, s.y_hat_static, s.nS, s.adv_cols, M,
-                        nullptr, 0, none, 0, din.hi, din.lo, din.pitch);
-      GANTTS_LAUNCH_CHECK("gather_planes_kernel(adv)");
+                        nullptr, 0, none, 0, fk.hi, fk.lo, fk.pitch);
+      GANTTS_LAUNCH_CHECK("gather_planes_kernel(fake)");
     }
     if (s.d_rnn() && (rc = discriminator_stack_fwd(s, stacked, nullptr, tape_in))) return rc;
+    if (half >= 0) return mlp_fwd_rows(&s.d, nullptr, 0, rows, r0, r1, L.d_out, 1, L.d_tape, L.d_tape_bytes, s.st);
     return mlp_fwd_impl(&s.d, nullptr, 0, rows, L.d_out, 1, L.d_tape, L.d_tape_bytes, s.stream, true);
   }
   const int dD = s.dD;
   if (stacked) {
-    gather_cols_list_kernel<<<blocks_1d(M * s.nA, 1024), 256, 0, s.st>>>(s.y, s.d_out, L.d_in + s.cond_w, dD, s.real_cols, M);
-    GANTTS_LAUNCH_CHECK("gather_cols_list_kernel(real)");
-    gather_cols_list_kernel<<<blocks_1d(M * s.nA, 1024), 256, 0, s.st>>>(s.y_hat_static, s.nS, L.d_in + M * dD + s.cond_w,
-                                                                          dD, s.adv_cols, M);
-    GANTTS_LAUNCH_CHECK("gather_cols_list_kernel(fake)");
-    for (int64_t half = 0; half < 2; ++half)
-      GANTTS_CUDA(cudaMemcpy2DAsync(L.d_in + half * M * dD, (size_t)dD * sizeof(float), s.x, (size_t)s.d_in * sizeof(float),
+    if (half != 1) {
+      gather_cols_list_kernel<<<blocks_1d(M * s.nA, 1024), 256, 0, s.st>>>(s.y, s.d_out, L.d_in + s.cond_w, dD, s.real_cols, M);
+      GANTTS_LAUNCH_CHECK("gather_cols_list_kernel(real)");
+    }
+    if (half != 0) {
+      gather_cols_list_kernel<<<blocks_1d(M * s.nA, 1024), 256, 0, s.st>>>(s.y_hat_static, s.nS, L.d_in + M * dD + s.cond_w,
+                                                                            dD, s.adv_cols, M);
+      GANTTS_LAUNCH_CHECK("gather_cols_list_kernel(fake)");
+    }
+    for (int64_t h = r0 / M; h < r1 / M; ++h)
+      GANTTS_CUDA(cudaMemcpy2DAsync(L.d_in + h * M * dD, (size_t)dD * sizeof(float), s.x, (size_t)s.d_in * sizeof(float),
                                     (size_t)s.cond_w * sizeof(float), (size_t)M, cudaMemcpyDeviceToDevice, s.st));
+    if (half >= 0) return mlp_fwd_rows(&s.d, L.d_in, dD, rows, r0, r1, L.d_out, 1, L.d_tape, L.d_tape_bytes, s.st);
   }
   if (s.d_rnn()) {
     if ((rc = discriminator_stack_fwd(s, stacked, L.d_in + (stacked ? 0 : M * dD), tape_in))) return rc;
@@ -1133,7 +1147,7 @@
   return gantts_mlp_fwd(&s.d, L.d_in + (stacked ? 0 : M * dD), dD, rows, L.d_out, 1, L.d_tape, L.d_tape_bytes, s.stream);
 }
 
-static int discriminator_bwd(Step& s, bool stacked, bool input_grad = true) {
+static int discriminator_bwd(Step& s, bool stacked, bool input_grad = true, bool fake_chain = false) {
   const StepLayout& L = s.L;
   const int64_t M = s.M, skip = stacked ? M : 0;
   float* const* gW = stacked ? s.pd.gW : nullptr;
@@ -1154,16 +1168,33 @@
     if ((rc = lstm_stack_bwd(k, stacked ? L.d_lstm.lengths : s.lengths, stacked ? 2 * s.B : s.B, s.T, s.seed, stacked,
                              input_grad ? &din : nullptr, s.st)))
       return rc;
-  } else if ((rc = mlp_bwd_impl(&s.d, L.g_dout, 1, L.d_out, 1, skip + M, L.d_tape, L.d_tape_bytes, gx, s.adv_window ? s.nS : s.dD,
-                                skip, gW, gb, 0, L.mlp_ws, L.mlp_ws_bytes, s.stream, s.adv_window ? 1 : -1, false,
-                                stacked ? s.side : nullptr))) {
-    return rc;
+  } else {
+    if (fake_chain && (rc = stream_wait(s.side, s.branch))) return rc;
+    if ((rc = mlp_bwd_impl(&s.d, L.g_dout, 1, L.d_out, 1, skip + M, L.d_tape, L.d_tape_bytes, gx, s.adv_window ? s.nS : s.dD,
+                           skip, gW, gb, 0, L.mlp_ws, L.mlp_ws_bytes, s.stream, s.adv_window ? 1 : -1, false,
+                           stacked ? s.side : nullptr, fake_chain ? M : 0)))
+      return rc;
   }
   if (s.adv_window || !input_grad) return GANTTS_OK;
   scatter_cols_list_add_kernel<<<blocks_1d(M * s.nA, 1024), 256, 0, s.st>>>(L.g_din + skip * s.dD + s.cond_w, s.dD,
                                                                              L.g_static, s.nS, s.adv_cols, M);
   GANTTS_LAUNCH_CHECK("scatter_cols_list_add_kernel");
   return GANTTS_OK;
+}
+
+static int discriminator_real_half(Step& s) {
+  const StepLayout& L = s.L;
+  int rc;
+  if ((rc = mlp_split_weights(&s.d, 2 * s.M, L.d_tape, L.d_tape_bytes, s.st))) return rc;
+  if ((rc = stream_wait(s.branch, s.st))) return rc;
+  Step b = s;
+  b.st = s.branch;
+  b.stream = s.branch;
+  if ((rc = discriminator_fwd(b, true, 0))) return rc;
+  if ((rc = launch_bce(L.d_out, L.mask, s.M, 1, 0, 0, L.scal + S_INV_T, L.g_dout, &L.red[R_REAL], nullptr, b.st)))
+    return rc;
+  return mlp_bwd_impl(&s.d, L.g_dout, 1, L.d_out, 1, 2 * s.M, L.d_tape, L.d_tape_bytes, nullptr, 0, 0, nullptr, nullptr,
+                      0, L.mlp_ws, L.mlp_ws_bytes, b.stream, -1, false, nullptr, 0, s.M);
 }
 
 }
@@ -1243,7 +1274,9 @@
   s.stream = stream;
   s.st = as_stream(stream);
   s.side = nullptr;
+  s.branch = nullptr;
   if ((g_side_bwd(c) || d_side_bwd(c)) && (rc = side_stream(&s.side))) return rc;
+  if (d_real_branch(c) && (rc = branch_stream(&s.branch))) return rc;
   layout(c, reinterpret_cast<char*>(al256(reinterpret_cast<uintptr_t>(workspace))), &s.L);
   const StepLayout& L = s.L;
   const int64_t M = s.M = (int64_t)B * T;
@@ -1315,6 +1348,11 @@
   if (phases & 1) {
     NvtxRange r1("gantts_gan_step/phase1: G fwd, MLPG, MGE, D fwd+bwd");
     if ((rc = step_prologue(s, inv_frames, d_only))) return rc;
+    const bool branch = s.has_d && d_real_branch(c);
+    if (branch) {
+      s.d.seed = gantts_gan_step_seed(seed, 1);
+      if ((rc = discriminator_real_half(s))) return rc;
+    }
     if ((rc = generator_fwd(s, true))) return rc;
     if ((rc = launch_sse(y_hat_static, nS, y, s.d_out, L.mask, M, nS, L.scal + S_MGE_SCALE, d_only ? nullptr : L.g_static, nS,
                          &L.red[R_MGE], st, &s.static_cols)))
@@ -1324,10 +1362,17 @@
       return rc;
     if (s.has_d) {
       s.d.seed = gantts_gan_step_seed(seed, 1);
-      if ((rc = discriminator_fwd(s, true))) return rc;
-      if ((rc = launch_bce(L.d_out, L.mask, M, 2, 0, 1, L.scal + S_INV_T, L.g_dout, &L.red[R_REAL], &L.red[R_FAKE], st)))
-        return rc;
-      if ((rc = discriminator_bwd(s, true, !d_only))) return rc;
+      if (branch) {
+        if ((rc = discriminator_fwd(s, true, 1))) return rc;
+        if ((rc = launch_bce(L.d_out + M, L.mask, M, 1, 1, 0, L.scal + S_INV_T, L.g_dout + M, &L.red[R_FAKE], nullptr,
+                             st)))
+          return rc;
+      } else {
+        if ((rc = discriminator_fwd(s, true))) return rc;
+        if ((rc = launch_bce(L.d_out, L.mask, M, 2, 0, 1, L.scal + S_INV_T, L.g_dout, &L.red[R_REAL], &L.red[R_FAKE], st)))
+          return rc;
+      }
+      if ((rc = discriminator_bwd(s, true, !d_only, branch))) return rc;
     }
   }
   if (d_only) {
diff --git a/gantts_b200/csrc/gemm_tc.cu b/gantts_b200/csrc/gemm_tc.cu
--- a/gantts_b200/csrc/gemm_tc.cu
+++ b/gantts_b200/csrc/gemm_tc.cu
@@ -600,6 +600,13 @@
   cur += plane_bytes(rows, cols);
   pl.lo = reinterpret_cast<__nv_bfloat16*>(cur);
   cur += plane_bytes(rows, cols);
+  return pl;
+}
+
+static Planes plane_rows(Planes pl, int64_t r0, int64_t r1) {
+  pl.hi += r0 * pl.pitch;
+  pl.lo += r0 * pl.pitch;
+  pl.rows = r1 - r0;
   return pl;
 }
 
diff --git a/gantts_b200/csrc/mlp_tc.cu b/gantts_b200/csrc/mlp_tc.cu
--- a/gantts_b200/csrc/mlp_tc.cu
+++ b/gantts_b200/csrc/mlp_tc.cu
@@ -160,7 +160,7 @@
                 const uint32_t* __restrict__ code, int64_t code_pitch, const float* __restrict__ w,
                 __nv_bfloat16* __restrict__ ghi, __nv_bfloat16* __restrict__ glo, int64_t gpitch,
                 float* __restrict__ partial, int64_t M, int K, int sigmoid, float dpos, float dneg, float dzero,
-                int want_gw) {
+                int want_gw, int want_gz) {
   __shared__ float ws[GEMV_MAX_K];
   __shared__ float gws[GEMV_THREADS / 32][GEMV_MAX_K + 1];
   for (int i = threadIdx.x; i < K; i += GEMV_THREADS) ws[i] = w[i];
@@ -189,6 +189,7 @@
         gws[wid][c] = fmaf(g, a0, gws[wid][c]);
         if (c + 1 < K) gws[wid][c + 1] = fmaf(g, a1, gws[wid][c + 1]);
       }
+      if (!want_gz) continue;
       const uint32_t cw = code[r * code_pitch + (c >> 4)];
       const uint32_t c0 = (cw >> (2 * (c & 15))) & 3u, c1 = (cw >> (2 * ((c + 1) & 15))) & 3u;
       const float v0 = g * ws[c] * ((c0 & 1u) ? dzero : ((c0 & 2u) ? dneg : dpos));
@@ -293,7 +294,7 @@
                     const uint32_t* __restrict__ code, int64_t code_pitch, const float* __restrict__ w,
                     __nv_bfloat16* __restrict__ ghi, __nv_bfloat16* __restrict__ glo, int64_t gpitch,
                     float* __restrict__ partial, int64_t M, int K, int sigmoid, float dpos, float dneg, float dzero,
-                    int want_gw) {
+                    int want_gw, int want_gz) {
   pdl_entry();
   __shared__ float gws[GEMV_THREADS / 32][GEMV_MAX_K + 1];
   const int lane = threadIdx.x & 31, wid = threadIdx.x >> 5;
@@ -332,7 +333,7 @@
             h[u][ch] = ldg_stream16(hi + r * pitch + c);
             l[u][ch] = ldg_stream16(lo + r * pitch + c);
           }
-          cw[u][ch] = __ldg(code + r * code_pitch + (c >> 4)) >> (2 * (c & 15));
+          if (want_gz) cw[u][ch] = __ldg(code + r * code_pitch + (c >> 4)) >> (2 * (c & 15));
         }
       }
     }
@@ -351,6 +352,7 @@
 #pragma unroll
           for (int j = 0; j < 8; ++j) gw[ch][j] = fmaf(g[u], a[j], gw[ch][j]);
         }
+        if (!want_gz) continue;
         uint32_t oh[4], ol[4];
 #pragma unroll
         for (int j = 0; j < 4; ++j) {
@@ -502,6 +504,85 @@
 namespace gantts {
 static int mlp_fwd_impl(const gantts_mlp_t* m, const float* x, int64_t x_rs, int64_t M, float* y, int64_t y_rs, void* tape,
                         size_t tape_bytes, void* stream, bool input_ready);
+static int mlp_split_weights(const gantts_mlp_t* m, int64_t M, void* tape, size_t tape_bytes, cudaStream_t st);
+static int mlp_fwd_rows(const gantts_mlp_t* m, const float* x, int64_t x_rs, int64_t M, int64_t r0, int64_t r1, float* y,
+                        int64_t y_rs, void* tape, size_t tape_bytes, cudaStream_t st);
+
+static int split_weights(const gantts_mlp_t* m, const MlpTape& t, cudaStream_t st) {
+  const int L = m->num_layers;
+  WeightSplitList wl;
+  wl.n = L;
+  wl.off[0] = 0;
+  for (int l = 0; l < L; ++l) {
+    wl.W[l] = m->W[l];
+    wl.N[l] = m->dims[l + 1];
+    wl.K[l] = m->dims[l];
+    wl.hi[l] = t.W[l].hi;
+    wl.lo[l] = t.W[l].lo;
+    wl.pitch[l] = t.W[l].pitch;
+    wl.thi[l] = t.Wt[l].hi;
+    wl.tlo[l] = t.Wt[l].lo;
+    wl.tpitch[l] = t.Wt[l].pitch;
+    wl.off[l + 1] = wl.off[l] + (int64_t)((m->dims[l + 1] + 31) / 32) * ((m->dims[l] + 31) / 32);
+  }
+  int nb = (int)wl.off[L];
+  if (nb > num_sms() * 8) nb = num_sms() * 8;
+  if (nb < 1) nb = 1;
+  GANTTS_PDL_LAUNCH((split_weights_kernel), nb, 256, 0, st, wl);
+  GANTTS_LAUNCH_CHECK("split_weights_kernel");
+  return GANTTS_OK;
+}
+
+static int fwd_layers(const gantts_mlp_t* m, const MlpTape& t, int64_t r0, int64_t r1, float* y, int64_t y_rs,
+                      cudaStream_t st) {
+  const int L = m->num_layers;
+  const int64_t M = r1 - r0;
+  y += r0 * y_rs;
+  int rc;
+  for (int l = 0; l < L; ++l) {
+    const Planes A = plane_rows(t.H[l], r0, r1);
+    EpiArgs e;
+    e.bias = m->b[l];
+    e.row0 = r0;
+    if (l < L - 1) {
+      const Planes O = plane_rows(t.H[l + 1], r0, r1);
+      e.epi = EPI_PLANES_FWD;
+      e.out_hi = O.hi;
+      e.out_lo = O.lo;
+      e.out_pitch = O.pitch;
+      e.code = t.code[l + 1] + r0 * t.code_pitch[l + 1];
+      e.code_pitch = t.code_pitch[l + 1];
+      e.act = GANTTS_ACT_LEAKY_DROPOUT;
+      e.slope = m->slope;
+      e.p = m->dropout_p;
+      e.seed = layer_seed(m->seed, l);
+    } else {
+      if (m->dims[L] == 1 && L >= 2 && m->dims[l] <= GEMV_MAX_K && (m->dims[l] & 1) == 0) {
+        const int Kl = m->dims[l], sg = m->last_act == GANTTS_ACT_SIGMOID;
+        if (Kl % 8 == 0 && Kl <= 256)
+          GANTTS_PDL_LAUNCH((gemv_fwd_vec_kernel<1, 4>), 2 * GEMV_BLOCKS, GEMV_THREADS, 0, st, A.hi, A.lo, A.pitch, m->W[l],
+                                                                          m->b[l], y, y_rs, M, Kl, sg);
+        else if (Kl % 8 == 0 && Kl <= 512)
+          gemv_fwd_vec_kernel<2, 2><<<2 * GEMV_BLOCKS, GEMV_THREADS, 0, st>>>(A.hi, A.lo, A.pitch, m->W[l],
+                                                                          m->b[l], y, y_rs, M, Kl, sg);
+        else if (Kl % 8 == 0)
+          gemv_fwd_vec_kernel<4, 1><<<2 * GEMV_BLOCKS, GEMV_THREADS, 0, st>>>(A.hi, A.lo, A.pitch, m->W[l],
+                                                                          m->b[l], y, y_rs, M, Kl, sg);
+        else
+          gemv_fwd_kernel<<<GEMV_BLOCKS, GEMV_THREADS, 0, st>>>(A.hi, A.lo, A.pitch, m->W[l], m->b[l], y,
+                                                                y_rs, M, Kl, sg);
+        GANTTS_LAUNCH_CHECK("gemv_fwd_kernel");
+        continue;
+      }
+      e.epi = EPI_F32;
+      e.C = y;
+      e.ldc = y_rs;
+      e.act = m->last_act;
+    }
+    if ((rc = launch_gemm_kk(A, t.W[l], e, st))) return rc;
+  }
+  return GANTTS_OK;
+}
 
 static int mlp_tape_input_planes(const gantts_mlp_t* m, int64_t M, void* tape, size_t tape_bytes, Planes* out) {
   int rc = check_mlp(m, M);
@@ -536,77 +617,46 @@
   cudaStream_t st = as_stream(stream);
   MlpTape t;
   carve_tape(m, M, reinterpret_cast<char*>((reinterpret_cast<uintptr_t>(tape) + 255) / 256 * 256), &t);
-  const int L = m->num_layers;
   if (!input_ready && (rc = launch_split(x, x_rs, M, m->dims[0], t.H[0], 0, st))) return rc;
-  {
-    WeightSplitList wl;
-    wl.n = L;
-    wl.off[0] = 0;
-    for (int l = 0; l < L; ++l) {
-      wl.W[l] = m->W[l];
-      wl.N[l] = m->dims[l + 1];
-      wl.K[l] = m->dims[l];
-      wl.hi[l] = t.W[l].hi;
-      wl.lo[l] = t.W[l].lo;
-      wl.pitch[l] = t.W[l].pitch;
-      wl.thi[l] = t.Wt[l].hi;
-      wl.tlo[l] = t.Wt[l].lo;
-      wl.tpitch[l] = t.Wt[l].pitch;
-      wl.off[l + 1] = wl.off[l] + (int64_t)((m->dims[l + 1] + 31) / 32) * ((m->dims[l] + 31) / 32);
-    }
-    int nb = (int)wl.off[L];
-    if (nb > num_sms() * 8) nb = num_sms() * 8;
-    if (nb < 1) nb = 1;
-    GANTTS_PDL_LAUNCH((split_weights_kernel), nb, 256, 0, st, wl);
-    GANTTS_LAUNCH_CHECK("split_weights_kernel");
-  }
-  for (int l = 0; l < L; ++l) {
-    EpiArgs e;
-    e.bias = m->b[l];
-    if (l < L - 1) {
-      e.epi = EPI_PLANES_FWD;
-      e.out_hi = t.H[l + 1].hi;
-      e.out_lo = t.H[l + 1].lo;
-      e.out_pitch = t.H[l + 1].pitch;
-      e.code = t.code[l + 1];
-      e.code_pitch = t.code_pitch[l + 1];
-      e.act = GANTTS_ACT_LEAKY_DROPOUT;
-      e.slope = m->slope;
-      e.p = m->dropout_p;
-      e.seed = layer_seed(m->seed, l);
-    } else {
-      if (m->dims[L] == 1 && L >= 2 && m->dims[l] <= GEMV_MAX_K && (m->dims[l] & 1) == 0) {
-        const int Kl = m->dims[l], sg = m->last_act == GANTTS_ACT_SIGMOID;
-        if (Kl % 8 == 0 && Kl <= 256)
-          GANTTS_PDL_LAUNCH((gemv_fwd_vec_kernel<1, 4>), 2 * GEMV_BLOCKS, GEMV_THREADS, 0, st, t.H[l].hi, t.H[l].lo, t.H[l].pitch, m->W[l],
-                                                                          m->b[l], y, y_rs, M, Kl, sg);
-        else if (Kl % 8 == 0 && Kl <= 512)
-          gemv_fwd_vec_kernel<2, 2><<<2 * GEMV_BLOCKS, GEMV_THREADS, 0, st>>>(t.H[l].hi, t.H[l].lo, t.H[l].pitch, m->W[l],
-                                                                          m->b[l], y, y_rs, M, Kl, sg);
-        else if (Kl % 8 == 0)
-          gemv_fwd_vec_kernel<4, 1><<<2 * GEMV_BLOCKS, GEMV_THREADS, 0, st>>>(t.H[l].hi, t.H[l].lo, t.H[l].pitch, m->W[l],
-                                                                          m->b[l], y, y_rs, M, Kl, sg);
-        else
-          gemv_fwd_kernel<<<GEMV_BLOCKS, GEMV_THREADS, 0, st>>>(t.H[l].hi, t.H[l].lo, t.H[l].pitch, m->W[l], m->b[l], y,
-                                                                y_rs, M, Kl, sg);
-        GANTTS_LAUNCH_CHECK("gemv_fwd_kernel");
-        continue;
-      }
-      e.epi = EPI_F32;
-      e.C = y;
-      e.ldc = y_rs;
-      e.act = m->last_act;
-    }
-    if ((rc = launch_gemm_kk(t.H[l], t.W[l], e, st))) return rc;
-  }
-  return GANTTS_OK;
+  if ((rc = split_weights(m, t, st))) return rc;
+  return fwd_layers(m, t, 0, M, y, y_rs, st);
+}
+
+static int gantts::mlp_split_weights(const gantts_mlp_t* m, int64_t M, void* tape, size_t tape_bytes, cudaStream_t st) {
+  int rc = check_mlp(m, M);
+  if (rc) return rc;
+  if (!tape || tape_bytes < gantts_mlp_tape_bytes(m, M)) {
+    set_error("mlp_split_weights: tape too small");
+    return GANTTS_E_WORKSPACE;
+  }
+  MlpTape t;
+  carve_tape(m, M, reinterpret_cast<char*>((reinterpret_cast<uintptr_t>(tape) + 255) / 256 * 256), &t);
+  return split_weights(m, t, st);
+}
+
+static int gantts::mlp_fwd_rows(const gantts_mlp_t* m, const float* x, int64_t x_rs, int64_t M, int64_t r0, int64_t r1,
+                                float* y, int64_t y_rs, void* tape, size_t tape_bytes, cudaStream_t st) {
+  int rc = check_mlp(m, M);
+  if (rc) return rc;
+  GANTTS_CHECK_ARG(r0 >= 0 && r0 < r1 && r1 <= M, "mlp_fwd_rows: bad row window [%lld, %lld) of %lld rows",
+                   (long long)r0, (long long)r1, (long long)M);
+  GANTTS_CHECK_ARG((!x || x_rs >= m->dims[0]) && y && y_rs >= m->dims[m->num_layers], "mlp_fwd_rows: bad pointers/strides");
+  if (!tape || tape_bytes < gantts_mlp_tape_bytes(m, M)) {
+    set_error("mlp_fwd_rows: tape too small");
+    return GANTTS_E_WORKSPACE;
+  }
+  MlpTape t;
+  carve_tape(m, M, reinterpret_cast<char*>((reinterpret_cast<uintptr_t>(tape) + 255) / 256 * 256), &t);
+  if (x && (rc = launch_split(x + r0 * x_rs, x_rs, r1 - r0, m->dims[0], plane_rows(t.H[0], r0, r1), 0, st))) return rc;
+  return fwd_layers(m, t, r0, r1, y, y_rs, st);
 }
 
 namespace gantts {
 static int mlp_bwd_impl(const gantts_mlp_t* m, const float* gy, int64_t gy_rs, const float* y, int64_t y_rs, int64_t M,
                         const void* tape, size_t tape_bytes, float* gx, int64_t gx_rs, int64_t gx_row0,
                         float* const* gW, float* const* gb, int accumulate, void* workspace, size_t workspace_bytes,
-                        void* stream, int gx_accumulate = -1, bool gy_planes_ready = false, cudaStream_t side = nullptr);
+                        void* stream, int gx_accumulate = -1, bool gy_planes_ready = false, cudaStream_t side = nullptr,
+                        int64_t chain_r0 = 0, int64_t chain_r1 = -1);
 static int mlp_bwd_gy_planes(const gantts_mlp_t* m, int64_t M, void* workspace, size_t workspace_bytes, Planes* out);
 }
 
@@ -634,11 +684,16 @@
                                 int64_t M, const void* tape, size_t tape_bytes, float* gx, int64_t gx_rs,
                                 int64_t gx_row0, float* const* gW, float* const* gb, int accumulate, void* workspace,
                                 size_t workspace_bytes, void* stream, int gx_accumulate, bool gy_planes_ready,
-                                cudaStream_t side) {
+                                cudaStream_t side, int64_t chain_r0, int64_t chain_r1) {
   if (gx_accumulate < 0) gx_accumulate = accumulate;
   int rc = check_mlp(m, M);
   GANTTS_CHECK_ARG(gx_row0 >= 0 && gx_row0 < M, "mlp_bwd: bad gx_row0");
   if (rc) return rc;
+  if (chain_r1 < 0) chain_r1 = M;
+  GANTTS_CHECK_ARG(chain_r0 >= 0 && chain_r0 < chain_r1 && chain_r1 <= M, "mlp_bwd: bad chain rows [%lld, %lld)",
+                   (long long)chain_r0, (long long)chain_r1);
+  const bool windowed = chain_r0 > 0 || chain_r1 < M;
+  GANTTS_CHECK_ARG(!windowed || !gy_planes_ready, "mlp_bwd: a row window needs gy, not gy planes");
   const int L = m->num_layers;
   GANTTS_CHECK_ARG(gy_planes_ready || (gy && gy_rs >= m->dims[L]), "mlp_bwd: bad gy");
   GANTTS_CHECK_ARG(!gy_planes_ready || (m->last_act == GANTTS_ACT_NONE && m->dims[L] > 1),
@@ -648,7 +703,8 @@
     set_error("mlp_bwd: tape too small");
     return GANTTS_E_WORKSPACE;
   }
-  size_t need = mlp_workspace_bytes(m, M, false, side != nullptr);
+  const bool per_layer = side != nullptr || windowed;
+  size_t need = mlp_workspace_bytes(m, M, false, per_layer);
   if (!workspace || workspace_bytes < need) {
     set_error("mlp_bwd: workspace too small (%zu < %zu)", workspace_bytes, need);
     return GANTTS_E_WORKSPACE;
@@ -661,7 +717,7 @@
   int maxd = 0;
   for (int l = 0; l <= L; ++l) maxd = m->dims[l] > maxd ? m->dims[l] : maxd;
   char* cur = reinterpret_cast<char*>((reinterpret_cast<uintptr_t>(workspace) + 255) / 256 * 256);
-  const int nbuf = mlp_grad_bufs(m, side != nullptr);
+  const int nbuf = mlp_grad_bufs(m, per_layer);
   char* gbuf[GANTTS_MAX_LAYERS > MLP_GRAD_BUFS ? GANTTS_MAX_LAYERS : MLP_GRAD_BUFS];
   for (int i = 0; i < nbuf; ++i) {
     gbuf[i] = cur;
@@ -684,22 +740,33 @@
     G = carve_planes(cg, M, K1);
     const float ks = m->dropout_p > 0.f ? 1.f / (1.f - m->dropout_p) : 1.f;
     const int want = (gW && gW[L - 1]) || (gb && gb[L - 1]);
+    auto gemv_bwd = [&](int64_t r0, int64_t r1, int gw, int gz, cudaStream_t s) {
+      const Planes H = plane_rows(t.H[L - 1], r0, r1), Gw = plane_rows(G, r0, r1);
 #define GANTTS_GEMV_BWD_ARGS                                                                                     \
-  gy, gy_rs, y, y_rs, t.H[L - 1].hi, t.H[L - 1].lo, t.H[L - 1].pitch, t.code[L - 1], t.code_pitch[L - 1],       \
-      m->W[L - 1], G.hi, G.lo, G.pitch, gemv_part, M, K1, m->last_act == GANTTS_ACT_SIGMOID ? 1 : 0, ks,        \
-      m->slope * ks, m->dropout_p > 0.f ? 0.f : m->slope, want
-    if (K1 % 8 == 0 && K1 <= 256)
-      GANTTS_PDL_LAUNCH((gemv_bwd_vec_kernel<1, 4>), GEMV_BLOCKS, GEMV_THREADS, 0, st, GANTTS_GEMV_BWD_ARGS);
-    else if (K1 % 8 == 0 && K1 <= 512)
-      gemv_bwd_vec_kernel<2, 2><<<GEMV_BLOCKS, GEMV_THREADS, 0, st>>>(GANTTS_GEMV_BWD_ARGS);
-    else if (K1 % 8 == 0)
-      gemv_bwd_vec_kernel<4, 1><<<GEMV_BLOCKS, GEMV_THREADS, 0, st>>>(GANTTS_GEMV_BWD_ARGS);
-    else
-      gemv_bwd_kernel<<<GEMV_BLOCKS, GEMV_THREADS, 0, st>>>(GANTTS_GEMV_BWD_ARGS);
+  gy + r0 * gy_rs, gy_rs, y ? y + r0 * y_rs : nullptr, y_rs, H.hi, H.lo, H.pitch,                              \
+      t.code[L - 1] + r0 * t.code_pitch[L - 1], t.code_pitch[L - 1], m->W[L - 1], Gw.hi, Gw.lo, Gw.pitch,       \
+      gemv_part, r1 - r0, K1, m->last_act == GANTTS_ACT_SIGMOID ? 1 : 0, ks, m->slope * ks,                     \
+      m->dropout_p > 0.f ? 0.f : m->slope, gw, gz
+      if (K1 % 8 == 0 && K1 <= 256)
+        GANTTS_PDL_LAUNCH((gemv_bwd_vec_kernel<1, 4>), GEMV_BLOCKS, GEMV_THREADS, 0, s, GANTTS_GEMV_BWD_ARGS);
+      else if (K1 % 8 == 0 && K1 <= 512)
+        gemv_bwd_vec_kernel<2, 2><<<GEMV_BLOCKS, GEMV_THREADS, 0, s>>>(GANTTS_GEMV_BWD_ARGS);
+      else if (K1 % 8 == 0)
+        gemv_bwd_vec_kernel<4, 1><<<GEMV_BLOCKS, GEMV_THREADS, 0, s>>>(GANTTS_GEMV_BWD_ARGS);
+      else
+        gemv_bwd_kernel<<<GEMV_BLOCKS, GEMV_THREADS, 0, s>>>(GANTTS_GEMV_BWD_ARGS);
 #undef GANTTS_GEMV_BWD_ARGS
-    GANTTS_LAUNCH_CHECK("gemv_bwd_kernel");
+      GANTTS_LAUNCH_CHECK("gemv_bwd_kernel");
+      return GANTTS_OK;
+    };
+    if (!windowed) {
+      if ((rc = gemv_bwd(0, M, want, 1, st))) return rc;
+    } else if ((rc = gemv_bwd(chain_r0, chain_r1, 0, 1, st))) {
+      return rc;
+    }
     if (want) {
       if ((rc = fork())) return rc;
+      if (windowed && (rc = gemv_bwd(0, M, 1, 0, ws))) return rc;
       GANTTS_PDL_LAUNCH((gemv_partial_reduce_kernel), (K1 + 1 + 31) / 32, 256, 0, ws, gemv_part, GEMV_BLOCKS, K1,
                                                                     gW ? gW[L - 1] : nullptr,
                                                                     gb ? gb[L - 1] : nullptr, accumulate);
@@ -707,11 +774,13 @@
     }
     l_start = L - 2;
   } else if (!gy_planes_ready) {
-    int64_t total = M * m->dims[L];
+    const int64_t rows = chain_r1 - chain_r0, total = rows * m->dims[L];
     int nb = (int)((total + 1023) / 1024);
     if (nb > num_sms() * 8) nb = num_sms() * 8;
     if (nb < 1) nb = 1;
-    grad_out_to_planes_kernel<<<nb, 256, 0, st>>>(gy, gy_rs, y, y_rs, M, m->dims[L], G.hi, G.lo, G.pitch,
+    const Planes Gw = plane_rows(G, chain_r0, chain_r1);
+    grad_out_to_planes_kernel<<<nb, 256, 0, st>>>(gy + chain_r0 * gy_rs, gy_rs, y ? y + chain_r0 * y_rs : nullptr, y_rs,
+                                                  rows, m->dims[L], Gw.hi, Gw.lo, Gw.pitch,
                                                   m->last_act == GANTTS_ACT_SIGMOID ? 1 : 0);
     GANTTS_LAUNCH_CHECK("grad_out_to_planes_kernel");
   }
@@ -728,29 +797,27 @@
     if (l > 0) {
       char* c1 = gbuf[(pp + 1) % nbuf];
       Planes Gn = carve_planes(c1, M, m->dims[l]);
+      const Planes O = plane_rows(Gn, chain_r0, chain_r1);
       EpiArgs e;
       e.epi = EPI_PLANES_BWD;
-      e.out_hi = Gn.hi;
-      e.out_lo = Gn.lo;
-      e.out_pitch = Gn.pitch;
-      e.code = t.code[l];
+      e.out_hi = O.hi;
+      e.out_lo = O.lo;
+      e.out_pitch = O.pitch;
+      e.code = t.code[l] + chain_r0 * t.code_pitch[l];
       e.code_pitch = t.code_pitch[l];
       e.slope = m->slope;
       e.p = m->dropout_p;
-      if ((rc = launch_gemm_kk(G, t.Wt[l], e, st))) return rc;
+      if ((rc = launch_gemm_kk(plane_rows(G, chain_r0, chain_r1), t.Wt[l], e, st))) return rc;
       G = Gn;
       pp = (pp + 1) % nbuf;
-    } else if (gx) {
+    } else if (gx && (gx_row0 > chain_r0 ? gx_row0 : chain_r0) < chain_r1) {
+      const int64_t g0 = gx_row0 > chain_r0 ? gx_row0 : chain_r0;
       EpiArgs e;
       e.epi = EPI_F32;
-      e.C = gx + gx_row0 * gx_rs;
+      e.C = gx + g0 * gx_rs;
       e.ldc = gx_rs;
       e.accumulate = gx_accumulate;
-      Planes Gs = G;
-      Gs.hi += gx_row0 * G.pitch;
-      Gs.lo += gx_row0 * G.pitch;
-      Gs.rows = G.rows - gx_row0;
-      if ((rc = launch_gemm_kk(Gs, t.Wt[0], e, st))) return rc;
+      if ((rc = launch_gemm_kk(plane_rows(G, g0, chain_r1), t.Wt[0], e, st))) return rc;
     }
   }
   if ((rc = flush_reduce(rl, accumulate, ws))) return rc;
```

Measured after the change: 17.05 million (median of 6 runs). +3.6%, better.
